# CompVis/ipoke

Measured on AMD Instinct MI355X. Metric: video-frames/sec (second-stage train step), higher is better.
Workload: dtype bf16; 1 GPU; plants_128 second_stage train, 16x3x128x128 clips, z=64, flow 2048 hidden (1.237 B params), per-GPU batch 20; global_batch=20, clip_frames=16, parallelism=dp1, weights=random init of the named architecture (no checkpoints offline)

## Files before the change

### include/ipoke_hip_dev.h

```cpp
#ifndef IPOKE_HIP_DEV_H
#define IPOKE_HIP_DEV_H

#include "ipoke_hip.h"

#ifdef __cplusplus
extern "C" {
#endif

int ipoke_conv_forward_repeat(const ipoke_conv_desc* d, int dtype, int n, void* stream);
int ipoke_set_dispatch_override(const char* name, int value);
enum { IPOKE_KERNEL_NONE = 0, IPOKE_KERNEL_IGEMM = 1, IPOKE_KERNEL_S8 = 2, IPOKE_KERNEL_HALO = 3, IPOKE_KERNEL_HALO16 = 4, IPOKE_KERNEL_C64 = 5, IPOKE_KERNEL_K8 = 6 };
int ipoke_last_conv_kernel(void);

int ipoke_spin_delay(int us, void* stream);

#define IPOKE_TAG_NT_SQUARE 1
#define IPOKE_TAG_TN_SQUARE 2
#define IPOKE_TAG_UNIT_FWD 3
#define IPOKE_TAG_UNIT_BWD 4
#define IPOKE_TAG_UNIT_INV 5
#define IPOKE_TAG_NN_SQUARE 6
#define IPOKE_TAG_CONV_BASE 16
#define IPOKE_TAG_WGRAD 32
int ipoke_timing_start(void);
int ipoke_timing_start_all(void);
int ipoke_timing_stop(const int* tags, int ntags, int* counts, double* mean_us);
int ipoke_timing_stop_ex(const int* tags, int ntags, int* counts, double* total_us, double* flops, double* bytes);

int ipoke_desc_sizes(int32_t* out, int n);

int ipoke_flow_test_inject_timeout(ipoke_flow* f, int which, void* stream);

int ipoke_gru_set_fused(int mode);

#ifdef __cplusplus
}
#endif
#endif
```

### ipoke_amd/_lib.py

```python
import ctypes
import os
from ctypes import CFUNCTYPE, POINTER, Structure, c_char_p, c_float, c_int, c_int32, c_int64, c_uint32, c_void_p

_HERE = os.path.dirname(os.path.abspath(__file__))
LIB_PATH = os.environ.get("IPOKE_LIB_PATH") or os.path.join(_HERE, "libipoke_hip.so")

F32, BF16 = 0, 1
ACT_NONE, ACT_ELU, ACT_RELU, ACT_LRELU02, ACT_TANH, ACT_SIGMOID = range(6)

DTYPES = {"f32": F32, "fp32": F32, "float32": F32, "bf16": BF16, "bfloat16": BF16}


class ConvDesc(Structure):
    _fields_ = [(n, c_int32) for n in ("NB", "Di", "Hi", "Wi", "Do", "Ho", "Wo", "kd", "kh", "kw", "sd", "sh", "sw",
                                       "pd", "ph", "pw", "transposed")] + [
        ("A", c_void_p), ("a_f32", c_int32),
        ("a_sn", c_int64), ("a_sd", c_int64), ("a_sh", c_int64), ("a_sw", c_int64), ("a_sc", c_int64),
        ("a_coff", c_int32), ("Kc_real", c_int32), ("Kc", c_int32),
        ("W", c_void_p), ("ldw", c_int32), ("Nout", c_int32),
        ("bias", c_void_p), ("act", c_int32), ("dact", c_void_p), ("ld_dact", c_int32), ("dact_act", c_int32),
        ("C", c_void_p), ("c_f32", c_int32), ("c_accumulate", c_int32), ("ldc", c_int64),
        ("c_coff", c_int32), ("c_cstride", c_int32), ("splitk", c_int32),
        ("c_scatter", c_int32), ("c_sn", c_int64), ("c_sh", c_int64), ("c_sw", c_int64), ("c_row0", c_int64),
        ("row_scale", c_void_p), ("rs_images", c_int32), ("rs_stride", c_int32), ("w_kmajor", c_int32), ("c_sd", c_int64),
# ... 148 lines not shown
    "ipoke_actnorm_logdet": (c_int, [_P, _P, c_int, c_int, _P, _P]),
    "ipoke_flow_nll": (c_int, [_P, _P, c_int, c_int, c_int, c_int, c_float, _P, _P, _P, _P]),
    "ipoke_adam_amsgrad_step": (c_int, [_P, _P, _P, _P, _P, c_int64, c_float, c_float, c_float, c_float, c_float, c_int,
                                        c_float, _P]),
    "ipoke_adam_amsgrad_step_grid": (c_int, [_P, _P, _P, _P, _P, c_int64, c_float, c_float, c_float, c_float, c_float, c_int,
                                             c_float, c_int, _P]),
    "ipoke_mcf_shadow_dims": (c_int, [c_int, c_int, c_int, POINTER(c_int32)]),
    "ipoke_mcf_fwd": (c_int, [POINTER(McfDesc), c_int, _P]),
    "ipoke_mcf_inv": (c_int, [POINTER(McfDesc), c_int, _P]),
    "ipoke_mcf_bwd": (c_int, [POINTER(McfDesc), c_int, _P]),
    "ipoke_macow_unit_supported": (c_int, [c_int, c_int, c_int]),
    "ipoke_macow_unit_xchg_bytes": (c_int64, [c_int, c_int]),
    "ipoke_macow_unit_fwd": (c_int, [POINTER(McfDesc), c_int, _P]),
    "ipoke_macow_unit_bwd": (c_int, [POINTER(McfDesc), c_int, _P]),
    "ipoke_macow_unit_inv": (c_int, [POINTER(McfDesc), c_int, _P]),
    "ipoke_relayout_job_size": (c_int, []),
    "ipoke_wn_job_size": (c_int, []),
    "ipoke_relayout_multi": (c_int, [_P, _P, _P, _P, c_int, c_int, _P, c_int, _P]),
    "ipoke_wn_scale_multi": (c_int, [_P, _P, _P, _P, c_int, c_int, _P]),
    "ipoke_wn_bwd_multi": (c_int, [_P, _P, _P, _P, c_int, c_int, _P]),
    "ipoke_groupnorm_workspace_floats": (c_int64, [c_int, c_int, c_int]),
    "ipoke_groupnorm": (c_int, [POINTER(NormDesc), c_int, _P]),
    "ipoke_add_act": (c_int, [_P, c_int, _P, c_int, _P, c_int, c_int64, c_int, c_int, c_int, _P]),
    "ipoke_gru_gates": (c_int, [_P, _P, c_int, _P, c_int, _P, c_int64, c_int, c_int, _P]),
    "ipoke_gru_update": (c_int, [_P, _P, _P, c_int, _P, c_int, c_int64, c_int, c_int, _P]),
    "ipoke_reparameterize": (c_int, [_P, c_int, _P, _P, _P, _P, c_int64, c_int, c_int, _P]),
    "ipoke_bilinear_cl": (c_int, [_P, _P, c_int, c_int, c_int, c_int, c_int, c_int, _P]),
    "ipoke_cl_to_nchw": (c_int, [_P, c_int, _P, c_int, c_int, c_int, c_int, _P]),
    "ipoke_nchw_to_cl": (c_int, [_P, _P, c_int, c_int, c_int, c_int, c_int, _P]),
    "ipoke_image_metrics_workspace_bytes": (c_int64, [c_int64, c_int, c_int]),
    "ipoke_psnr_ssim": (c_int, [_P, _P, c_int64, c_int, c_int, _P, _P, _P]),
    "ipoke_clip_to_cl4": (c_int, [_P, c_int64, c_int64, c_int64, c_int64, c_int64, c_int, c_int, c_int, c_int, c_int, c_int, _P, c_int, _P]),
    "ipoke_groupnorm_stats": (c_int, [_P, c_int, c_int, c_int, c_int, c_int, c_float, _P, c_int, _P]),
    "ipoke_groupnorm_stats_offset": (c_int64, [c_int, c_int, c_int]),
    "ipoke_groupnorm_bwd_workspace_floats": (c_int64, [c_int, c_int, c_int, c_int]),
    "ipoke_groupnorm_bwd": (c_int, [POINTER(NormBwdDesc), c_int, _P]),
    "ipoke_groupnorm_bwd_rs_workspace_floats": (c_int64, [c_int, c_int, c_int]),
    "ipoke_act_bwd": (c_int, [_P, c_int, _P, c_int, _P, c_int, c_int64, c_int, c_int, c_int, c_int, _P]),
    "ipoke_colsum_workspace_floats": (c_int64, [c_int64, c_int]),
    "ipoke_colsum": (c_int, [_P, c_int, c_int64, c_int, c_int, _P, c_int, _P, c_int, _P]),
    "ipoke_gru_update_bwd": (c_int, [_P, _P, _P, c_int, _P, c_int, _P, _P, _P, c_int, c_int64, c_int, c_int, _P]),
    "ipoke_gru_gates_bwd": (c_int, [_P, _P, c_int, _P, c_int, _P, _P, _P, c_int, c_int64, c_int, c_int, _P]),
    "ipoke_conv_weight_operand": (c_int, [_P, c_int, c_int, c_int, c_int, _P, _P, c_int, c_int, _P]),
    "ipoke_conv_weight_operand_multi": (c_int, [POINTER(c_void_p), POINTER(c_void_p), POINTER(c_int32), c_int, c_int, _P]),
    "ipoke_spectral_workspace_floats": (ctypes.c_long, [c_int, c_int, c_int]),
    "ipoke_spectral_sigma": (c_int, [_P, c_int, c_int, c_int, c_int, _P, _P, c_int, ctypes.c_float, _P, _P, _P, _P]),
    "ipoke_spectral_bwd": (c_int, [_P, c_int, c_int, c_int, c_int, _P, _P, _P, _P, _P]),
    "ipoke_spectral_bwd_workspace_floats": (ctypes.c_long, []),
    "ipoke_sn_job_size": (c_int, []),
    "ipoke_sn_jobs_upload": (c_int, [_P, c_int, _P, _P]),
    "ipoke_spectral_sigma_multi": (c_int, [_P, c_int, c_int, c_int, c_int, c_float, _P]),
    "ipoke_adam_multi": (c_int, [_P, _P, _P, _P, _P, c_int, ctypes.c_float, ctypes.c_float, ctypes.c_float, ctypes.c_float,
                                 ctypes.c_float, c_int, ctypes.c_float, _P]),
    "ipoke_maxpool3d_fwd": (c_int, [_P, _P, c_int, _P, c_int, _P, c_int, _P]),
    "ipoke_maxpool3d_bwd": (c_int, [_P, _P, c_int, _P, _P, c_int, c_int, _P]),
    "ipoke_avgpool_rows": (c_int, [_P, c_int, _P, c_int, c_int64, c_int, c_int, c_int, _P]),
    "ipoke_avgpool_rows_bwd": (c_int, [_P, c_int, _P, c_int, c_int64, c_int, c_int, c_int, _P]),
    "ipoke_groupnorm_jvp": (c_int, [_P, c_int, _P, c_int, _P, c_int, _P, c_int, _P, c_int, _P, c_int, c_int, c_int, c_int, c_int, c_float,
                                    _P, c_int, _P]),
    "ipoke_groupnorm_jvp_bwd": (c_int, [_P, c_int, _P, c_int, _P, c_int, _P, c_int, _P, c_int, _P, c_int, _P, c_int, _P, _P,
                                        c_int, c_int, c_int, c_int, c_int, c_float, _P, c_int, _P]),
    "ipoke_groupnorm_jvp_workspace_floats": (ctypes.c_long, [c_int, c_int]),
    "ipoke_gather_rows": (c_int, [_P, c_int, _P, _P, c_int, c_int64, c_int, c_int, _P]),
    "ipoke_l1_pair": (c_int, [_P, c_int, _P, c_int, c_int64, c_int, c_float, _P, _P, c_int, c_int, _P]),
    "ipoke_kl_loss": (c_int, [_P, _P, c_int64, c_int, _P, _P, _P, _P]),
    "ipoke_reparam_bwd": (c_int, [_P, c_int, _P, _P, _P, _P, _P, c_int, c_int64, c_int, c_int, _P]),
    "ipoke_l1_loss": (c_int, [_P, c_int, _P, c_int, c_int, c_int, c_int64, c_float, _P, _P, c_int, _P, _P]),
    "ipoke_l1_loss_partials": (ctypes.c_long, []),
    "ipoke_relayout_multi_range": (c_int, [_P, _P, _P, _P, c_int, c_int, c_int, _P, c_int, _P]),
    "ipoke_wn_scale_multi_range": (c_int, [_P, _P, _P, _P, c_int, c_int, c_int, c_int, _P]),
    "ipoke_flow_prepare_weights_range": (c_int, [_P, _P, _P, c_int64, c_int64, _P]),
    "ipoke_flow_set_native_adam": (c_int, [_P, _P, _P, _P, c_float, c_float, c_float, c_float, c_float, c_int, c_float, c_int]),
    "ipoke_flow_adam_range": (c_int, [_P, _P, _P, _P, _P, _P, _P, c_int64, c_int64, c_float, c_float, c_float, c_float, c_float, c_int,
                                      c_float, c_int, _P]),
    "ipoke_adam_tile_job_size": (c_int, []),
    "ipoke_adam_seg_size": (c_int, []),
    "ipoke_adam_amsgrad_shadow_tiles": (c_int, [_P, _P, _P, _P, _P, _P, _P, c_int, c_int, c_int, c_float, c_float, c_float, c_float, c_float,
                                                c_int, c_float, c_int, c_int, _P]),
    "ipoke_adam_amsgrad_cast_tiles": (c_int, [_P, _P, _P, _P, _P, _P, _P, c_int, c_int, c_int, c_float, c_float, c_float, c_float, c_float,
                                              c_int, c_float, c_int, c_int, _P]),
    "ipoke_adam_amsgrad_segments": (c_int, [_P, _P, _P, _P, _P, _P, c_int, c_int, c_int64, c_int64, c_float, c_float, c_float, c_float,
                                            c_float, c_int, c_float, c_int, _P]),
    "ipoke_wn_bwd_multi_range": (c_int, [_P, _P, _P, _P, c_int, c_int, c_int, c_int, _P]),
    "ipoke_flow_backward_pieces": (c_int, [_P, _P, _P, _P, _P, _P, c_int, _P, _P, _P, c_int, _P, GRAD_READY_FN, _P, _P]),
    "ipoke_video_to_cl": (c_int, [_P, c_int64, c_int64, c_int64, c_int64, c_int64, c_int, c_int, c_int, c_int, c_int, _P, c_int, c_int, c_int,
                                  c_int, _P, _P]),
    "ipoke_min_reset": (c_int, [_P, _P]),
    "ipoke_denorm_if_negative": (c_int, [_P, c_int64, c_int, c_int, c_int, c_int, _P, _P]),
    "ipoke_pool3d_same": (c_int, [_P, _P, c_int, _P, c_int, c_int, _P]),
    "ipoke_pool_rows_weighted": (c_int, [_P, c_int, _P, c_int, c_int64, c_int, c_int, _P, c_int, _P]),
    "ipoke_activation_moments": (c_int, [_P, c_int, c_int, _P, _P, _P, _P]),
    "ipoke_flow_resize": (c_int, [_P, _P, c_int, c_int, c_int, c_int, c_int, c_int, c_float, _P]),
    "ipoke_poke_workspace_bytes": (c_int64, [c_int, c_int, c_int, c_int, c_int]),
    "ipoke_poke_simulate": (c_int, [_P, c_int, c_int, c_int, c_int, c_int, c_int, c_int, _P, _P, _P, _P, _P, _P, _P, _P]),
    "ipoke_timing_start": (c_int, []),
    "ipoke_timing_start_all": (c_int, []),
    "ipoke_timing_stop": (c_int, [POINTER(c_int), c_int, POINTER(c_int), POINTER(ctypes.c_double)]),
    "ipoke_timing_stop_ex": (c_int, [POINTER(c_int), c_int, POINTER(c_int), POINTER(ctypes.c_double), POINTER(ctypes.c_double),
                                     POINTER(ctypes.c_double)]),
    "ipoke_flow_create": (c_int, [POINTER(FlowConfig), POINTER(c_void_p)]),
    "ipoke_flow_destroy": (None, [_P]),
    "ipoke_flow_piece_ranges": (c_int, [_P, c_int, POINTER(c_int64), c_int]),
    "ipoke_flow_handoff_timeouts": (c_int, [_P, POINTER(c_uint32)]),
    "ipoke_flow_side_stream": (c_void_p, [_P]),
    "ipoke_flow_test_inject_timeout": (c_int, [_P, c_int, _P]),
    "ipoke_conv_wgrad_splitm": (c_int, [_P, c_int, c_int]),
    "ipoke_conv_acc_scratch_bytes": (c_int64, [c_int, c_int, c_int]),
    "ipoke_conv_acc_scratch_init": (c_int, [_P, _P]),
    "ipoke_flow_param_count": (c_int64, [_P]),
    "ipoke_flow_index_count": (c_int64, [_P]),
    "ipoke_flow_tensor_count": (c_int32, [_P]),
    "ipoke_flow_op_count": (c_int32, [_P]),
    "ipoke_flow_tensor_info": (c_int, [_P, c_int, c_char_p, c_int, POINTER(c_int64), POINTER(c_int32), POINTER(c_int64),
                                       POINTER(c_int32)]),
    "ipoke_flow_shadow_bytes": (c_int64, [_P]),
    "ipoke_flow_set_graph": (c_int, [_P, c_int]),
    "ipoke_flow_float_buffer_count": (c_int64, [_P]),
    "ipoke_flow_set_float_buffers": (c_int, [_P, _P]),
    "ipoke_lu_job_size": (c_int, []),
    "ipoke_lu_prepare": (c_int, [_P, _P, _P, _P, c_int, _P]),
    "ipoke_lu_apply": (c_int, [_P, _P, c_int64, c_int, c_int, _P, c_int, _P]),
    "ipoke_lu_wgrad": (c_int, [_P, _P, c_int, c_int, c_int, _P, _P, _P, _P, _P, _P, _P]),
    "ipoke_flow_op_info": (c_int, [_P, c_int, POINTER(c_int64)]),
    "ipoke_flow_shadow_base": (c_int64, [_P]),
    "ipoke_flow_workspace_bytes": (c_int64, [_P, c_int, c_int]),
    "ipoke_flow_prepare_weights": (c_int, [_P, _P, _P, _P]),
    "ipoke_flow_forward": (c_int, [_P, _P, _P, _P, _P, _P, c_int, _P, _P, _P, c_int, _P]),
    "ipoke_flow_init_forward": (c_int, [_P, _P, _P, _P, c_int, _P, _P, _P, _P]),
    "ipoke_flow_reverse": (c_int, [_P, _P, _P, _P, _P, _P, c_int, _P, _P, _P]),
    "ipoke_flow_backward": (c_int, [_P, _P, _P, _P, _P, _P, c_int, _P, _P, _P, _P]),
}

_lib = None


def lib():
    global _lib
    if _lib is None:
        if not os.path.exists(LIB_PATH):
            raise RuntimeError(
                f"{LIB_PATH} not found: the HIP extension is not built. ipoke_amd has no CPU fallback; "
                "run `make -C ipoke_amd/csrc` (or __graft_entry__.build()) first.")
        import torch
        handle = ctypes.CDLL(LIB_PATH)
        for name, (res, args) in SIGNATURES.items():
            fn = getattr(handle, name)
            fn.restype = res
            fn.argtypes = args
        _lib = handle
    return _lib


def check(rc):
    if rc != 0:
        msg = lib().ipoke_last_error()
        raise RuntimeError(f"libipoke_hip call failed ({rc}): {msg.decode() if msg else '?'}")


def ptr(t):
    if t is None:
        return None
    return c_void_p(t.data_ptr())


def current_stream():
    import torch
# ... 23 lines not shown
```

### ipoke_amd/csrc/flow_engine.hip

```cpp
#include <functional>
#include <memory>
#include <vector>
#include <string>
#include <cstring>

#include "common.h"

namespace ipoke {

enum OpType { OP_ACTNORM = 0, OP_MCF = 1, OP_NICE = 2, OP_LU = 3 };
enum TensorKind { TK_PARAM = 0, TK_IDX_FWD = 1, TK_IDX_BWD = 2, TK_FLAG = 3, TK_FBUF = 4 };

struct TensorInfo {
  std::string name;
  int64_t offset;
  std::vector<int64_t> shape;
  int kind;
};

struct Op {
  int type = 0;
  int C = 0;
  int c0 = 0, Cn = 0;
  int64_t p_ls = -1, p_bias = -1, idx_fwd = -1, idx_bwd = -1;
  int order = 0;
  int64_t p_w1 = -1, p_b = -1, p_g = -1, p_v = -1;
  int Cp = 0, K1p = 0, K2p = 0, K3p = 0, Hq = 0, H = 0;
  int64_t sh_w1 = -1, sh_w1t = -1, sh_w2 = -1, sh_w2t = -1;
  int64_t wn_off = -1;
  int cin = 0, cout = 0, z_off = 0, z_stride = 1, t_off = 0, t_stride = 1;
  int64_t p_c1 = -1, p_c2 = -1;
  int Kc1 = 0, Kc3 = 0;
  int64_t sh_c1 = -1, sh_c1t = -1, sh_c2 = -1, sh_c2t = -1, sh_c3 = -1, sh_c3t = -1;
  int64_t ws_a = -1, ws_b = -1, ws_c = -1, ws_d = -1, ws_e = -1, ws_f = -1, ws_g = -1;
  int slot = -1;
  int mcf_idx = -1;
  int nice_idx = -1;
  int hidK = 0;
  int level = 0;
  int fuse_act = -1;
  bool fused = false;
  bool unit_head = false;
  int unit_of = -1;
  int lu_idx = -1;
  int an_next = -1;
  int an_prev = -1;
  int pair_unit = -1;
};

struct RelayoutJobH {
  long src_off, s_n, s_k, dstA, dstB, scale_off;
  int taps, n_real, k_real, A_rows_pad, A_inner_pad, B_rows_pad, B_inner_pad, B_rows_real, tile, tiles_k, block_start, frag_tiled;
};
struct WnJobH { long v_off, g_off, out_off; int rows, K, row_start; };
struct AdamTileJobH { long src_off, dstA, dstB; int N, K, tile_start, pad; };
struct AdamSegH { long off, len; };
struct LsRefH { long off; int C; };
struct LuJobH { long p_l, p_u, p_logs, b_perm, b_sign, b_lmask, b_umask, b_eye, w_off; int C, pad; };

}

using namespace ipoke;

struct ipoke_flow {
  ipoke_flow_config cfg;
  int esz = 2, e16 = 8, ks = 32;
  std::vector<TensorInfo> tensors;
  std::vector<Op> ops;
  int64_t n_params = 0, n_perm = 0, n_fbuf = 0;
  std::vector<LuJobH> lujobs; void* d_lujobs = nullptr; const float* fbuf = nullptr;
  int64_t shadow_elems = 0;
  int64_t wn_rows = 0;
  int nslots = 0;
  int n_mcf = 0;
  int tab_B = 0; void* d_w1tab = nullptr; void* d_w2tab = nullptr; void* d_redtab = nullptr; int n_red = 0;
  void* d_ntab[3] = {nullptr, nullptr, nullptr};
  int n_nice = 0;
  std::vector<RelayoutJobH> rjobs; int rblocks = 0;
  std::vector<AdamTileJobH> ajobs; int atiles = 0;
  std::vector<RelayoutJobH> rjobs2; int rblocks2 = 0;
  std::vector<AdamSegH> asegs;
  void* d_ajobs = nullptr; void* d_rjobs2 = nullptr; void* d_rblockjob2 = nullptr; void* d_asegs = nullptr;
  std::vector<WnJobH> wjobs;
  std::vector<LsRefH> lsrefs;
  void* d_rjobs = nullptr; void* d_wjobs = nullptr; void* d_lsrefs = nullptr; void* d_rblockjob = nullptr;
  hipStream_t side = nullptr;
  std::vector<hipStream_t> lanes;
  int n_lanes = 1;
  std::vector<hipEvent_t> events; size_t ev_next = 0;
  bool use_side = true;
  struct GraphEntry { std::vector<uintptr_t> key; hipGraph_t graph = nullptr; hipGraphExec_t exec = nullptr; int state = 0; uint64_t used = 0; };
  std::vector<GraphEntry> graphs; hipStream_t cap = nullptr; bool use_graph = false; uint64_t tick = 0;
  struct Unit { int64_t p_lo, p_hi; int wj_lo, wj_hi, row_lo, row_hi; int kind; int op_lo, op_hi; int64_t p2_lo = -1, p2_hi = -1; };
  std::vector<Unit> units;
  std::vector<int> red_first;
  int last_fwd_B = 0; bool have_saved = false;
  int P = 64;
  int unit_split = 1; void* d_xchg = nullptr;
  bool coupling_fuse = false; void* d_cxchg = nullptr;
  void* d_acc = nullptr; int64_t acc_bytes = 0;
  unsigned* h_tmo = nullptr; hipEvent_t pass_ev = nullptr; hipStream_t pass_stream = nullptr; bool pass_recorded = false, pass_unchecked = false;
  int64_t xchg_bytes = 0;
  bool mcf_xop = false;
  bool c2_straight = false;
  struct NativeAdam { bool on = false; float* m = nullptr; float* v = nullptr; float* vmax = nullptr; float lr = 0, beta1 = 0, beta2 = 0, eps = 0, wd = 0,
                      grad_scale = 1; int step = 0, max_blocks = 0; } nadam;
};

namespace {

int64_t align_up(int64_t v, int64_t a) { return (v + a - 1) / a * a; }

struct Builder {
  ipoke_flow& f;
  explicit Builder(ipoke_flow& fl) : f(fl) {}
  int64_t add_param(const std::string& name, std::vector<int64_t> shape) {
    int64_t n = 1; for (auto s : shape) n *= s;
    const int64_t off = f.n_params;
    f.tensors.push_back({name, off, shape, TK_PARAM});
    f.n_params = align_up(off + n, 4);
    return off;
  }
  int64_t add_idx(const std::string& name, int C, int kind) {
    const int64_t off = f.n_perm;
    f.tensors.push_back({name, off, {C}, kind});
    f.n_perm += C;
    return off;
  }
  void add_flag(const std::string& name) { f.tensors.push_back({name, -1, {}, TK_FLAG}); }
  int64_t add_fbuf(const std::string& name, std::vector<int64_t> shape) {
    int64_t n = 1; for (auto s : shape) n *= s;
    const int64_t off = f.n_fbuf;
    f.tensors.push_back({name, off, shape, TK_FBUF});
    f.n_fbuf = align_up(off + n, 4);
    return off;
  }
  void lu(const std::string& pfx, int C) {
    Op op; op.type = OP_LU; op.C = C; op.lu_idx = (int)f.lujobs.size();
    LuJobH j{};
    j.C = C;
    j.p_l = add_param(pfx + ".l", {C, C}); j.p_u = add_param(pfx + ".u", {C, C}); j.p_logs = add_param(pfx + ".log_s", {C});
    j.b_perm = add_fbuf(pfx + ".permutated", {C, C}); j.b_sign = add_fbuf(pfx + ".sign_s", {C});
    j.b_lmask = add_fbuf(pfx + ".lmask", {C, C}); j.b_umask = add_fbuf(pfx + ".umask", {C, C}); j.b_eye = add_fbuf(pfx + ".eye", {C, C});
    j.w_off = (long)op.lu_idx * 4 * 64 * 64;
    f.lujobs.push_back(j);
    f.lsrefs.push_back({j.p_logs, C});
    f.ops.push_back(op);
  }
  int64_t add_shadow(int64_t elems) {
    const int64_t off = f.shadow_elems;
    f.shadow_elems = align_up(off + elems, 64);
    return off;
  }
  void relayout_pair(long src, long s_n, long s_k, int taps, int n_real, int k_real, long scale, long dstA, int A_rows_pad,
                     int A_inner_pad, long dstB, int B_rows_pad, int B_inner_pad, int B_rows_real, int frag_tiled = 0) {
    const int tile = taps == 1 ? 64 : 32;
    const int n_ext = std::max(A_rows_pad, B_inner_pad), k_ext = std::max(A_inner_pad, B_rows_pad);
    const int tiles_n = (n_ext + tile - 1) / tile, tiles_k = (k_ext + tile - 1) / tile;
    RelayoutJobH j{src, s_n, s_k, dstA, dstB, scale, taps, n_real, k_real, A_rows_pad, A_inner_pad, B_rows_pad, B_inner_pad,
                   B_rows_real, tile, tiles_k, f.rblocks, frag_tiled};
    f.rjobs.push_back(j);
    f.rblocks += tiles_n * tiles_k;
    const bool fusable = taps == 1 && scale < 0 && !frag_tiled && s_k == 1 && s_n == k_real && n_real % 64 == 0 && k_real % 64 == 0 &&
                         A_rows_pad == n_real && A_inner_pad == k_real && B_rows_pad == k_real && B_inner_pad == n_real &&
                         B_rows_real == k_real;
    if (fusable) {
      f.ajobs.push_back({src, dstA, dstB, n_real, k_real, f.atiles, 0});
      f.atiles += (n_real / 64) * (k_real / 64);
    } else {
      j.block_start = f.rblocks2;
      f.rjobs2.push_back(j);
      f.rblocks2 += tiles_n * tiles_k;
    }
  }

  void actnorm(const std::string& pfx, int C_active, int c0, int Cn, const std::string* shuffle_pfx) {
    Op op; op.type = OP_ACTNORM; op.C = C_active; op.c0 = c0; op.Cn = Cn;
    if (!pfx.empty()) {
      op.p_ls = add_param(pfx + ".log_scale", {Cn, 1, 1});
      op.p_bias = add_param(pfx + ".bias", {Cn, 1, 1});
      add_flag(pfx + ".initialized");
      f.lsrefs.push_back({(long)op.p_ls, Cn});
    }
    if (shuffle_pfx) {
      op.idx_fwd = add_idx(*shuffle_pfx + ".forward_shuffle_idx", Cn, TK_IDX_FWD);
      op.idx_bwd = add_idx(*shuffle_pfx + ".backward_shuffle_idx", Cn, TK_IDX_BWD);
    }
    f.ops.push_back(op);
  }

  void mcf(const std::string& pfx, int C, int order) {
    const int Cc = f.cfg.cond_channels;
    Op op; op.type = OP_MCF; op.C = C; op.order = order;
    const int kh = order < 2 ? f.cfg.kernel_h : f.cfg.kernel_w, kw = order < 2 ? f.cfg.kernel_w : f.cfg.kernel_h;
    op.H = 4 * C;
    op.Cp = round_up(C, f.ks);
    op.K1p = 6 * op.Cp;
    op.K2p = round_up(op.H + Cc, f.ks);
    op.K3p = round_up(2 * C, f.ks);
    op.Hq = round_up(op.H, f.ks);
    const int K2 = op.H + Cc;
    op.p_w1 = add_param(pfx + ".net.shift_conv.weight", {op.H, C, kh, kw});
    add_flag(pfx + ".net.conv1x1.initialized");
    op.p_b = add_param(pfx + ".net.conv1x1.conv.bias", {2 * C});
    op.p_g = add_param(pfx + ".net.conv1x1.conv.weight_g", {2 * C, 1, 1, 1});
    op.p_v = add_param(pfx + ".net.conv1x1.conv.weight_v", {2 * C, K2, 1, 1});
    op.wn_off = f.wn_rows;
    f.wjobs.push_back({(long)op.p_v, (long)op.p_g, (long)op.wn_off, 2 * C, K2, (int)f.wn_rows});
    f.wn_rows += 2 * C;
    const int Hr = round_up(op.H, 16), N2r = round_up(2 * C, 16), Cr = round_up(C, 16);
    op.sh_w1 = add_shadow((int64_t)Hr * op.K1p);
    op.sh_w1t = add_shadow((int64_t)Cr * 6 * op.Hq);
    op.sh_w2 = add_shadow((int64_t)N2r * op.K2p);
    op.sh_w2t = add_shadow((int64_t)Hr * op.K3p);
    relayout_pair(op.p_w1, (long)C * 6, 6, 6, op.H, C, -1, op.sh_w1, Hr, op.Cp, op.sh_w1t, Cr, op.Hq, C, 1);
    relayout_pair(op.p_v, K2, 1, 1, 2 * C, K2, op.wn_off, op.sh_w2, N2r, op.K2p, op.sh_w2t, Hr, op.K3p, op.H, 1);
    op.slot = f.nslots++;
    op.mcf_idx = f.n_mcf++;
    f.ops.push_back(op);
  }

  void nice(const std::string& pfx, int C, bool skip, bool up, int factor) {
    const int hid = f.cfg.hidden;
    Op op; op.type = OP_NICE; op.C = C;
    op.cout = C / factor; op.cin = C - op.cout;
    if (skip && (C % 2 == 1)) skip = false;
    if (!skip) {
      const int z1 = up ? op.cin : op.cout;
      if (up) { op.z_off = 0; op.t_off = z1; } else { op.z_off = z1; op.t_off = 0; }
      op.z_stride = op.t_stride = 1;
    } else {
      op.z_stride = op.t_stride = 2;
      if (up) { op.z_off = 0; op.t_off = 1; } else { op.z_off = 1; op.t_off = 0; }
    }
    op.Kc1 = round_up(op.cin, f.e16);
    op.Kc3 = round_up(2 * op.cout, f.e16);
    const int hidK = hid + (f.cfg.condition_nice ? f.cfg.cond_channels : 0);
    op.hidK = hidK;
    op.p_c1 = add_param(pfx + ".net.conv1.weight", {hid, op.cin, 3, 3});
    op.p_c2 = add_param(pfx + ".net.conv2.weight", {hid, hid, 1, 1});
    add_flag(pfx + ".net.conv3.initialized");
    op.p_b = add_param(pfx + ".net.conv3.conv.bias", {2 * op.cout});
    op.p_g = add_param(pfx + ".net.conv3.conv.weight_g", {2 * op.cout, 1, 1, 1});
    op.p_v = add_param(pfx + ".net.conv3.conv.weight_v", {2 * op.cout, hidK, 3, 3});
    op.wn_off = f.wn_rows;
    f.wjobs.push_back({(long)op.p_v, (long)op.p_g, (long)op.wn_off, 2 * op.cout, hidK * 9, (int)f.wn_rows});
    f.wn_rows += 2 * op.cout;
    const int N3 = 2 * op.cout;
    op.sh_c1 = add_shadow((int64_t)hid * 9 * op.Kc1);
    op.sh_c1t = add_shadow((int64_t)op.cin * 9 * hid);
    op.sh_c2 = add_shadow((int64_t)hid * hid);
    op.sh_c2t = f.c2_straight ? -1 : add_shadow((int64_t)hid * hid);
    op.sh_c3 = add_shadow((int64_t)N3 * 9 * hidK);
// ... 331 lines not shown
    const int rmul = op.unit_of >= 0 || op.pair_unit >= 0 ? f->unit_split : 1;
    if (op.type == OP_MCF) {
      const McfGeom g = mcf_geom(op.order);
      w1[op.mcf_idx] = {f->mcf_xop ? (long)op.ws_e : (long)(plan.state0 + (int64_t)i * plan.state_stride), (long)op.ws_d, (long)op.p_w1, g.kh,
                        g.kw, -g.oy, -g.ox};
      w2[op.mcf_idx] = {(long)op.ws_a, (long)op.ws_c, (long)op.p_v, 1, 1, 0, 0};
      red.push_back({dbp, (long)op.p_b, 2 * op.C, 2 * op.C, rmul, 0});
    } else if (op.type == OP_NICE) {
      nt[0][op.nice_idx] = {(long)op.ws_g, (long)op.ws_f, (long)op.p_c1, 3, 3, 1, 1};
      nt[1][op.nice_idx] = {(long)op.ws_a, (long)op.ws_e, (long)op.p_c2, 1, 1, 0, 0, (long)op.sh_c2};
      nt[2][op.nice_idx] = {(long)op.ws_b, (long)op.ws_d, (long)op.p_v, 3, 3, 1, 1};
      red.push_back({dbp, (long)op.p_b, 2 * op.cout, 2 * op.cout, rmul, 0});
    } else if (op.p_ls >= 0) {
      red.push_back({dbp, (long)op.p_ls, 2 * op.Cn, op.Cn, rmul, 0});
      red.push_back({dbp + op.Cn, (long)op.p_bias, 2 * op.Cn, op.Cn, rmul, 0});
    }
  }
  drop_graphs(f);
  f->red_first[f->ops.size()] = (int)red.size();
  if (f->d_w1tab) { (void)hipFree(f->d_w1tab); (void)hipFree(f->d_w2tab); (void)hipFree(f->d_redtab); }
  for (int k = 0; k < 3; ++k) {
    if (f->d_ntab[k]) (void)hipFree(f->d_ntab[k]);
    IPK_HIP(hipMalloc(&f->d_ntab[k], nt[k].size() * sizeof(WgEntryH)));
    IPK_HIP(hipMemcpy(f->d_ntab[k], nt[k].data(), nt[k].size() * sizeof(WgEntryH), hipMemcpyHostToDevice));
  }
  IPK_HIP(hipMalloc(&f->d_w1tab, w1.size() * sizeof(WgEntryH)));
  IPK_HIP(hipMalloc(&f->d_w2tab, w2.size() * sizeof(WgEntryH)));
  IPK_HIP(hipMalloc(&f->d_redtab, red.size() * sizeof(RedEntryH)));
  IPK_HIP(hipMemcpy(f->d_w1tab, w1.data(), w1.size() * sizeof(WgEntryH), hipMemcpyHostToDevice));
  IPK_HIP(hipMemcpy(f->d_w2tab, w2.data(), w2.size() * sizeof(WgEntryH), hipMemcpyHostToDevice));
  IPK_HIP(hipMemcpy(f->d_redtab, red.data(), red.size() * sizeof(RedEntryH), hipMemcpyHostToDevice));
  f->n_red = (int)red.size();
  f->tab_B = B;
  return IPOKE_OK;
}

std::vector<std::pair<int, int>> backward_pieces(const ipoke_flow* f, int npieces) {
  std::vector<std::pair<int, int>> pieces;
  const int U = (int)f->units.size();
  int64_t total = 0;
  for (const auto& u : f->units) total += u.p_hi - u.p_lo;
  const int np = npieces < 1 ? 1 : (npieces > U ? U : npieces);
  static double ta = -1, tb = -1;
  if (ta < 0) {
    ta = 0.5; tb = 0.25;
    if (const char* e = getenv("IPOKE_PIECE_TAPER")) { double a = 0, b = 0; if (sscanf(e, "%lf,%lf", &a, &b) == 2 && a > 0 && b > 0) { ta = a; tb = b; } }
  }
  std::vector<double> w((size_t)np, 1.0);
  if (np >= 4) { w[(size_t)np - 2] = ta; w[(size_t)np - 1] = tb; }
  double wsum = 0; for (double x : w) wsum += x;
  int hi = U - 1;
  int64_t acc = 0; double target_acc = 0;
  int64_t done = 0;
  for (int u = U - 1; u >= 0; --u) {
    acc += f->units[u].p_hi - f->units[u].p_lo;
    const int idx = (int)pieces.size();
    const int left = np - idx;
    const double want = (double)total * (target_acc + w[(size_t)(idx < np ? idx : np - 1)]) / wsum;
    if (u == 0 || (left > 1 && ((double)(done + acc) >= want || u == left - 1))) {
      pieces.push_back({u, hi}); hi = u - 1; done += acc; acc = 0; target_acc += w[(size_t)(idx < np ? idx : np - 1)];
    }
  }
  return pieces;
}
void piece_param_ranges(const ipoke_flow* f, int lvl_lo, int lvl_hi, int64_t p0[3], int64_t p1[3]) {
  for (int k = 0; k < 3; ++k) { p0[k] = -1; p1[k] = -1; }
  for (int u = lvl_lo; u <= lvl_hi; ++u) {
    const auto& un = f->units[u];
    const int k = un.kind;
    if (p0[k] < 0) p0[k] = un.p_lo;
    p1[k] = un.p_hi;
    if (un.p2_lo >= 0) { if (p0[2] < 0) p0[2] = un.p2_lo; p1[2] = un.p2_hi; }
  }
}

hipEvent_t next_event(ipoke_flow* f) {
  hipEvent_t e = f->events[f->ev_next];
  f->ev_next = (f->ev_next + 1) % f->events.size();
  return e;
}

}

extern "C" int ipoke_flow_create(const ipoke_flow_config* cfg, ipoke_flow** out) {
  IPK_REQUIRE(cfg && out, "null argument");
  IPK_REQUIRE(cfg->dtype == IPOKE_F32 || cfg->dtype == IPOKE_BF16, "bad dtype");
  IPK_REQUIRE(cfg->n_levels >= 1 && cfg->n_levels <= 32 && cfg->n_levels < cfg->factor, "num_steps must be shorter than factor");
  IPK_REQUIRE(cfg->z_channels % cfg->factor == 0 && cfg->z_channels <= 64, "flow_in_channels must be a multiple of factor, <= 64");
  IPK_REQUIRE((cfg->z_channels / cfg->factor) % 2 == 0, "channel step must be even (skip split)");
  IPK_REQUIRE(cfg->kernel_h == 2 && cfg->kernel_w == 3, "kernel_size must be [2,3] (shipped configs)");
  IPK_REQUIRE(cfg->hidden % 32 == 0 && cfg->cond_channels % 32 == 0, "hidden / cond widths must be multiples of 32");
  std::unique_ptr<ipoke_flow> f(new ipoke_flow());
  f->cfg = *cfg;
  f->esz = cfg->dtype == IPOKE_BF16 ? 2 : 4; f->e16 = 16 / f->esz; f->ks = 64 / f->esz;
  {
    const char* cs = getenv("IPOKE_C2_STRAIGHT");
    f->c2_straight = cfg->dtype == IPOKE_BF16 && cfg->hidden % 64 == 0 && !(cs && cs[0] == '0');
  }
  int rc = build(*f); if (rc) return rc;
  {
    int64_t pos = 0;
    for (size_t k = 0; k < f->ajobs.size(); ++k) {
      IPK_REQUIRE(f->ajobs[k].src_off >= pos, "fused tensors must be in parameter order");
      if (f->ajobs[k].src_off > pos) f->asegs.push_back({(long)pos, (long)(f->ajobs[k].src_off - pos)});
      pos = f->ajobs[k].src_off + (int64_t)f->ajobs[k].N * f->ajobs[k].K;
    }
    if (pos < f->n_params) f->asegs.push_back({(long)pos, (long)(f->n_params - pos)});
    for (size_t k = 1; k < f->rjobs.size(); ++k) IPK_REQUIRE(f->rjobs[k].src_off > f->rjobs[k - 1].src_off, "relayout jobs must be in parameter order");
  }
  const char* env = getenv("IPOKE_NO_SIDE_STREAM");
  f->use_side = !(env && env[0] == '1');
  const char* gr = getenv("IPOKE_GRAPH");
  f->use_graph = gr && gr[0] == '1';
  const char* ln = getenv("IPOKE_LANES");
  f->n_lanes = ln ? atoi(ln) : 1;
  if (f->n_lanes < 1) f->n_lanes = 1;
  if (f->n_lanes > kMaxLanes) f->n_lanes = kMaxLanes;
  {
    const char* us = getenv("IPOKE_UNIT_SPLIT");
    f->unit_split = us ? atoi(us) : kDefaultUnitSplit;
    if (f->unit_split != 2 && f->unit_split != 4) f->unit_split = 1;
    if (f->n_lanes > 1 || cfg->dtype != IPOKE_BF16) f->unit_split = 1;
  }
  f->coupling_fuse = f->n_lanes == 1 && cfg->dtype == IPOKE_BF16 && ipoke_conv3x3_coupling_splitk(64, cfg->hidden, cfg->dtype) > 0;
  {
    const char* up = getenv("IPOKE_UNIT_PAIR");
    const bool on = f->unit_split > 1 && f->n_lanes == 1 && (up ? atoi(up) != 0 : true);
    for (size_t h = 2; on && h < f->ops.size(); ++h) {
      const Op& u = f->ops[h]; Op& an = f->ops[h - 1]; Op& cp = f->ops[h - 2];
      if (u.unit_head && an.type == OP_ACTNORM && an.an_prev == (int)h - 2 && cp.type == OP_NICE && an.c0 == 0 && an.Cn == u.C &&
          cp.cout <= 32 && cp.t_off + (cp.cout - 1) * cp.t_stride < u.C) {
        an.pair_unit = (int)h; cp.pair_unit = (int)h;
      }
    }
  }
  *out = f.release();
  return IPOKE_OK;
}

static int ensure_device(ipoke_flow* f) {
  if (f->d_rjobs) return IPOKE_OK;
  if (f->unit_split > 1 && !f->d_xchg) {
    const int64_t nb = ipoke_macow_unit_xchg_bytes(f->cfg.max_batch, f->unit_split);
    IPK_HIP(hipMalloc(&f->d_xchg, nb));
    IPK_HIP(hipMemset(f->d_xchg, 0, nb));
    f->xchg_bytes = nb;
  }
  if (!f->d_acc) {
    static const bool atomics = getenv("IPOKE_DGRAD_ATOMICS") != nullptr;
    if (!atomics) {
      f->acc_bytes = ipoke_conv_acc_scratch_bytes(f->cfg.max_batch * f->P, 64, 32);
      IPK_HIP(hipMalloc(&f->d_acc, (size_t)f->acc_bytes));
      int rc = ipoke_conv_acc_scratch_init(f->d_acc, nullptr); if (rc) return rc;
      IPK_HIP(hipDeviceSynchronize());
    }
  }
  if (!f->h_tmo) {
    IPK_HIP(hipHostMalloc(reinterpret_cast<void**>(&f->h_tmo), 64, hipHostMallocMapped));
    std::memset(f->h_tmo, 0, 64);
    IPK_HIP(hipEventCreateWithFlags(&f->pass_ev, hipEventDisableTiming));
  }
  if (f->coupling_fuse && !f->d_cxchg) {
    IPK_HIP(hipMalloc(&f->d_cxchg, (size_t)ipoke_conv3x3_coupling_xchg_bytes()));
    int rc = ipoke_conv3x3_coupling_xchg_init(f->d_cxchg, nullptr); if (rc) return rc;
    IPK_HIP(hipDeviceSynchronize());
  }
  IPK_REQUIRE((int)sizeof(RelayoutJobH) == ipoke_relayout_job_size() && (int)sizeof(WnJobH) == ipoke_wn_job_size(),
              "job table layout mismatch");
  IPK_HIP(hipMalloc(&f->d_rjobs, f->rjobs.size() * sizeof(RelayoutJobH)));
  IPK_HIP(hipMemcpy(f->d_rjobs, f->rjobs.data(), f->rjobs.size() * sizeof(RelayoutJobH), hipMemcpyHostToDevice));
  {
    std::vector<int32_t> bj((size_t)f->rblocks);
    for (size_t k = 0; k < f->rjobs.size(); ++k) {
      const int b0 = f->rjobs[k].block_start, b1 = k + 1 < f->rjobs.size() ? f->rjobs[k + 1].block_start : f->rblocks;
      for (int b = b0; b < b1; ++b) bj[b] = (int32_t)k;
    }
    IPK_HIP(hipMalloc(&f->d_rblockjob, bj.size() * sizeof(int32_t)));
    IPK_HIP(hipMemcpy(f->d_rblockjob, bj.data(), bj.size() * sizeof(int32_t), hipMemcpyHostToDevice));
  }
  IPK_REQUIRE((int)sizeof(AdamTileJobH) == ipoke_adam_tile_job_size() && (int)sizeof(AdamSegH) == ipoke_adam_seg_size(), "Adam table layout mismatch");
  if (!f->ajobs.empty()) {
    IPK_HIP(hipMalloc(&f->d_ajobs, f->ajobs.size() * sizeof(AdamTileJobH)));
    IPK_HIP(hipMemcpy(f->d_ajobs, f->ajobs.data(), f->ajobs.size() * sizeof(AdamTileJobH), hipMemcpyHostToDevice));
  }
  if (!f->asegs.empty()) {
    IPK_HIP(hipMalloc(&f->d_asegs, f->asegs.size() * sizeof(AdamSegH)));
    IPK_HIP(hipMemcpy(f->d_asegs, f->asegs.data(), f->asegs.size() * sizeof(AdamSegH), hipMemcpyHostToDevice));
  }
  if (!f->rjobs2.empty()) {
    IPK_HIP(hipMalloc(&f->d_rjobs2, f->rjobs2.size() * sizeof(RelayoutJobH)));
    IPK_HIP(hipMemcpy(f->d_rjobs2, f->rjobs2.data(), f->rjobs2.size() * sizeof(RelayoutJobH), hipMemcpyHostToDevice));
    std::vector<int32_t> bj((size_t)f->rblocks2);
    for (size_t k = 0; k < f->rjobs2.size(); ++k) {
      const int b0 = f->rjobs2[k].block_start, b1 = k + 1 < f->rjobs2.size() ? f->rjobs2[k + 1].block_start : f->rblocks2;
      for (int b = b0; b < b1; ++b) bj[b] = (int32_t)k;
    }
    IPK_HIP(hipMalloc(&f->d_rblockjob2, bj.size() * sizeof(int32_t)));
    IPK_HIP(hipMemcpy(f->d_rblockjob2, bj.data(), bj.size() * sizeof(int32_t), hipMemcpyHostToDevice));
  }
  IPK_HIP(hipMalloc(&f->d_wjobs, f->wjobs.size() * sizeof(WnJobH)));
  IPK_HIP(hipMemcpy(f->d_wjobs, f->wjobs.data(), f->wjobs.size() * sizeof(WnJobH), hipMemcpyHostToDevice));
  if (!f->lujobs.empty()) {
    IPK_REQUIRE((int)sizeof(LuJobH) == ipoke_lu_job_size(), "LU job table layout mismatch");
    IPK_HIP(hipMalloc(&f->d_lujobs, f->lujobs.size() * sizeof(LuJobH)));
    IPK_HIP(hipMemcpy(f->d_lujobs, f->lujobs.data(), f->lujobs.size() * sizeof(LuJobH), hipMemcpyHostToDevice));
  }
  IPK_HIP(hipMalloc(&f->d_lsrefs, f->lsrefs.size() * sizeof(LsRefH)));
  IPK_HIP(hipMemcpy(f->d_lsrefs, f->lsrefs.data(), f->lsrefs.size() * sizeof(LsRefH), hipMemcpyHostToDevice));
  {
    int least = 0, greatest = 0;
    IPK_HIP(hipDeviceGetStreamPriorityRange(&least, &greatest));
    static const bool flat = getenv("IPOKE_SIDE_FLAT_PRIORITY") != nullptr;
    IPK_HIP(hipStreamCreateWithPriority(&f->side, hipStreamNonBlocking, flat ? 0 : least));
  }
  IPK_HIP(hipStreamCreateWithFlags(&f->cap, hipStreamNonBlocking));
  f->lanes.resize(kMaxLanes - 1);
  for (auto& l : f->lanes) IPK_HIP(hipStreamCreateWithFlags(&l, hipStreamNonBlocking));
  f->events.resize(256);
  for (auto& e : f->events) IPK_HIP(hipEventCreateWithFlags(&e, hipEventDisableTiming));
  return IPOKE_OK;
}

extern "C" void ipoke_flow_destroy(ipoke_flow* f) {
  if (!f) return;
  if (f->d_rjobs) (void)hipFree(f->d_rjobs);
  if (f->d_wjobs) (void)hipFree(f->d_wjobs);
  if (f->d_lsrefs) (void)hipFree(f->d_lsrefs);
  if (f->d_lujobs) (void)hipFree(f->d_lujobs);
  if (f->d_rblockjob) (void)hipFree(f->d_rblockjob);
  if (f->d_ajobs) (void)hipFree(f->d_ajobs);
  if (f->d_asegs) (void)hipFree(f->d_asegs);
  if (f->d_rjobs2) (void)hipFree(f->d_rjobs2);
  if (f->d_rblockjob2) (void)hipFree(f->d_rblockjob2);
  if (f->d_w1tab) (void)hipFree(f->d_w1tab);
  for (int k = 0; k < 3; ++k) if (f->d_ntab[k]) (void)hipFree(f->d_ntab[k]);
  if (f->d_w2tab) (void)hipFree(f->d_w2tab);
  if (f->d_redtab) (void)hipFree(f->d_redtab);
  if (f->d_xchg) (void)hipFree(f->d_xchg);
  if (f->d_cxchg) (void)hipFree(f->d_cxchg);
  if (f->d_acc) (void)hipFree(f->d_acc);
  if (f->pass_ev) (void)hipEventDestroy(f->pass_ev);
  if (f->h_tmo) (void)hipHostFree(f->h_tmo);
  for (auto e : f->events) (void)hipEventDestroy(e);
  drop_graphs(f);
  if (f->side) (void)hipStreamDestroy(f->side);
  if (f->cap) (void)hipStreamDestroy(f->cap);
  for (auto l : f->lanes) if (l) (void)hipStreamDestroy(l);
  delete f;
}

extern "C" int ipoke_flow_piece_ranges(const ipoke_flow* f, int npieces, int64_t* ranges, int max_ranges) {
  IPK_REQUIRE(f != nullptr && (ranges != nullptr || max_ranges == 0), "bad arguments");
  const std::vector<std::pair<int, int>> pieces = backward_pieces(f, npieces);
  int n = 0;
  for (size_t i = 0; i < pieces.size(); ++i) {
    int64_t p0[3], p1[3];
    piece_param_ranges(f, pieces[i].first, pieces[i].second, p0, p1);
    for (int kind = 0; kind < 3; ++kind) {
      if (p0[kind] < 0 || p1[kind] <= p0[kind]) continue;
      if (n < max_ranges) { ranges[3 * n] = (int64_t)i; ranges[3 * n + 1] = p0[kind]; ranges[3 * n + 2] = p1[kind]; }
      ++n;
    }
  }
  return n;
}

extern "C" void* ipoke_flow_side_stream(ipoke_flow* f) {
  if (!f || ensure_device(f) != IPOKE_OK) return nullptr;
  return reinterpret_cast<void*>(f->side);
}
extern "C" int64_t ipoke_flow_param_count(const ipoke_flow* f) { return f ? f->n_params : -1; }
extern "C" int64_t ipoke_flow_index_count(const ipoke_flow* f) { return f ? f->n_perm : -1; }
extern "C" int ipoke_flow_set_graph(ipoke_flow* f, int enable) {
  IPK_REQUIRE(f != nullptr, "null flow handle");
  f->use_graph = enable != 0;
  return IPOKE_OK;
}
extern "C" int64_t ipoke_flow_float_buffer_count(const ipoke_flow* f) { return f ? f->n_fbuf : -1; }
extern "C" int ipoke_flow_set_float_buffers(ipoke_flow* f, const float* fbuf_dev) {
  IPK_REQUIRE(f != nullptr, "null flow handle");
  f->fbuf = fbuf_dev;
  return IPOKE_OK;
}
extern "C" int32_t ipoke_flow_tensor_count(const ipoke_flow* f) { return f ? (int32_t)f->tensors.size() : -1; }
extern "C" int32_t ipoke_flow_op_count(const ipoke_flow* f) { return f ? (int32_t)f->ops.size() : -1; }
extern "C" int ipoke_flow_tensor_info(const ipoke_flow* f, int i, char* name, int name_cap, int64_t* offset, int32_t* ndim,
                                      int64_t* shape4, int32_t* kind) {
  IPK_REQUIRE(f && i >= 0 && i < (int)f->tensors.size() && name && offset && ndim && shape4 && kind, "bad arguments");
  const TensorInfo& t = f->tensors[i];
  IPK_REQUIRE((int)t.name.size() + 1 <= name_cap, "name buffer too small");
  std::memcpy(name, t.name.c_str(), t.name.size() + 1);
  *offset = t.offset; *ndim = (int32_t)t.shape.size(); *kind = t.kind;
  for (int k = 0; k < 4; ++k) shape4[k] = k < (int)t.shape.size() ? t.shape[k] : 1;
  return IPOKE_OK;
}
extern "C" int ipoke_flow_op_info(const ipoke_flow* f, int i, int64_t* out32) {
  IPK_REQUIRE(f && out32 && i >= 0 && i < (int)f->ops.size(), "bad arguments");
  const Op& o = f->ops[i];
  const int64_t v[32] = {o.type, o.C, o.c0, o.Cn, o.p_ls, o.p_bias, o.idx_fwd, o.idx_bwd, o.order, o.p_w1, o.p_b, o.p_g, o.p_v,
                         o.sh_w1, o.sh_w1t, o.sh_w2, o.sh_w2t, o.wn_off, o.cin, o.cout, o.z_off, o.z_stride, o.t_off, o.t_stride,
                         o.p_c1, o.p_c2, o.sh_c1, o.sh_c1t, o.sh_c2, o.sh_c2t, o.sh_c3, o.sh_c3t};
  for (int k = 0; k < 32; ++k) out32[k] = v[k];
  return IPOKE_OK;
}
extern "C" int64_t ipoke_flow_shadow_base(const ipoke_flow* f) { return f ? 2 * align_up(f->wn_rows, 64) * 4 : -1; }

extern "C" int64_t ipoke_flow_shadow_bytes(const ipoke_flow* f) {
  if (!f) return -1;
  return 2 * align_up(f->wn_rows, 64) * 4 + f->shadow_elems * f->esz;
}
extern "C" int64_t ipoke_flow_workspace_bytes(ipoke_flow* f, int B, int training) {
  if (!f || B < 1) return -1;
  return make_plan(*f, B, training ? 1 : 0).bytes;
}
// ... 21 lines not shown
    const int row0 = f->wjobs[w0].row_start;
    const int row1 = w1 < (int)f->wjobs.size() ? f->wjobs[w1].row_start : (int)f->wn_rows;
    int rc = ipoke_wn_scale_multi_range(params, wn_scale, wn_inv, f->d_wjobs, w0, w1 - w0, row0, row1 - row0, stream);
    if (rc) return rc;
  }
  const std::vector<RelayoutJobH>& jobs = skip_fused ? f->rjobs2 : f->rjobs;
  const int nblocks = skip_fused ? f->rblocks2 : f->rblocks;
  int j0 = 0, j1 = 0;
  while (j0 < (int)jobs.size() && jobs[j0].src_off < begin) ++j0;
  j1 = j0;
  while (j1 < (int)jobs.size() && jobs[j1].src_off < end) ++j1;
  if (j1 > j0) {
    const int b0 = jobs[j0].block_start;
    const int b1 = j1 < (int)jobs.size() ? jobs[j1].block_start : nblocks;
    void* sh = reinterpret_cast<unsigned char*>(shadow) + 2 * align_up(f->wn_rows, 64) * 4;
    return ipoke_relayout_multi_range(params, sh, wn_scale, skip_fused ? f->d_rjobs2 : f->d_rjobs, (int)jobs.size(), b0, b1 - b0,
                                      reinterpret_cast<const int32_t*>(skip_fused ? f->d_rblockjob2 : f->d_rblockjob), f->cfg.dtype, stream);
  }
  return IPOKE_OK;
}

extern "C" int ipoke_flow_set_native_adam(ipoke_flow* f, float* m, float* v, float* vmax, float lr, float beta1, float beta2, float eps,
                                          float weight_decay, int step, float grad_scale, int max_blocks) {
  IPK_REQUIRE(f != nullptr, "null flow handle");
  ipoke_flow::NativeAdam& A = f->nadam;
  A.on = m != nullptr;
  if (!A.on) return IPOKE_OK;
  IPK_REQUIRE(v && vmax && step >= 1, "bad optimizer state");
  A.m = m; A.v = v; A.vmax = vmax; A.lr = lr; A.beta1 = beta1; A.beta2 = beta2; A.eps = eps; A.wd = weight_decay; A.step = step;
  A.grad_scale = grad_scale; A.max_blocks = max_blocks;
  return IPOKE_OK;
}

extern "C" int ipoke_flow_prepare_weights_range(ipoke_flow* f, const float* params, void* shadow, int64_t begin, int64_t end,
                                                void* stream) {
  IPK_REQUIRE(f && params && shadow && begin >= 0 && end >= begin, "bad arguments");
  { int rc0 = ensure_device(f); if (rc0) return rc0; }
  return prepare_range(f, params, shadow, begin, end, false, stream);
}

static int adam_range(ipoke_flow* f, float* params, const float* grads, float* m, float* v, float* vmax, void* shadow, int64_t begin, int64_t end,
                      float lr, float beta1, float beta2, float eps, float weight_decay, int step, float grad_scale, int max_blocks, void* stream,
                      bool skip_tiles = false);

extern "C" int ipoke_flow_adam_range(ipoke_flow* f, float* params, const float* grads, float* m, float* v, float* vmax, void* shadow,
                                     int64_t begin, int64_t end, float lr, float beta1, float beta2, float eps, float weight_decay,
                                     int step, float grad_scale, int max_blocks, void* stream) {
  IPK_REQUIRE(f && params && grads && m && v && vmax && shadow && begin >= 0 && end >= begin && end <= f->n_params, "bad arguments");
  { int rc0 = ensure_device(f); if (rc0) return rc0; }
  return adam_range(f, params, grads, m, v, vmax, shadow, begin, end, lr, beta1, beta2, eps, weight_decay, step, grad_scale, max_blocks, stream);
}

static int adam_range(ipoke_flow* f, float* params, const float* grads, float* m, float* v, float* vmax, void* shadow, int64_t begin, int64_t end,
                      float lr, float beta1, float beta2, float eps, float weight_decay, int step, float grad_scale, int max_blocks, void* stream,
                      bool skip_tiles) {
  if (end == begin) return IPOKE_OK;
  int a0 = 0, a1 = 0;
  while (a0 < (int)f->ajobs.size() && f->ajobs[a0].src_off < begin) ++a0;
  a1 = a0;
  while (a1 < (int)f->ajobs.size() && f->ajobs[a1].src_off < end) ++a1;
  if (a1 > a0 && !skip_tiles) {
    IPK_REQUIRE(f->ajobs[a1 - 1].src_off + (int64_t)f->ajobs[a1 - 1].N * f->ajobs[a1 - 1].K <= end, "range must cover whole tensors");
    const int t0 = f->ajobs[a0].tile_start, t1 = a1 < (int)f->ajobs.size() ? f->ajobs[a1].tile_start : f->atiles;
    void* sh = reinterpret_cast<unsigned char*>(shadow) + 2 * align_up(f->wn_rows, 64) * 4;
    int rc = f->c2_straight
        ? ipoke_adam_amsgrad_cast_tiles(params, grads, m, v, vmax, sh, f->d_ajobs, (int)f->ajobs.size(), t0, t1 - t0, lr, beta1, beta2,
                                        eps, weight_decay, step, grad_scale, max_blocks, f->cfg.dtype, stream)
        : ipoke_adam_amsgrad_shadow_tiles(params, grads, m, v, vmax, sh, f->d_ajobs, (int)f->ajobs.size(), t0, t1 - t0, lr, beta1, beta2,
                                          eps, weight_decay, step, grad_scale, max_blocks, f->cfg.dtype, stream);
    if (rc) return rc;
  }
  int s0 = 0, s1 = 0;
  while (s0 < (int)f->asegs.size() && f->asegs[s0].off + f->asegs[s0].len <= begin) ++s0;
  s1 = s0;
  while (s1 < (int)f->asegs.size() && f->asegs[s1].off < end) ++s1;
  if (s1 > s0) {
    int per = max_blocks > 0 ? max_blocks / (s1 - s0) : 16;
    if (per < 2) per = 2; if (per > 32) per = 32;
    int rc = ipoke_adam_amsgrad_segments(params, grads, m, v, vmax, f->d_asegs, s0, s1 - s0, begin, end, lr, beta1, beta2, eps, weight_decay,
                                         step, grad_scale, per, stream);
    if (rc) return rc;
  }
  return prepare_range(f, params, shadow, begin, end, true, stream);
}

static int make_lanes(const Ctx& full, int want, std::vector<Ctx>& lanes) {
  ipoke_flow* f = full.f;
  int n = want < 1 ? 1 : want;
  if (n > kMaxLanes) n = kMaxLanes;
  if (n > full.B) n = full.B;
  lanes.clear();
  int b0 = 0;
  for (int k = 0; k < n; ++k) {
    const int nb = (full.B - b0 + (n - k) - 1) / (n - k);
    Ctx c = full;
    c.b0 = b0; c.B = nb; c.M = (int64_t)nb * f->P; c.Bfull = full.B; c.lane = k;
    c.s = k == 0 ? full.s : f->lanes[k - 1];
    lanes.push_back(c);
    b0 += nb;
  }
  return IPOKE_OK;
}
static int fork_lanes(ipoke_flow* f, hipStream_t from, const std::vector<Ctx>& lanes) {
  if (lanes.size() < 2) return IPOKE_OK;
  hipEvent_t e = next_event(f);
  IPK_HIP(hipEventRecord(e, from));
  for (size_t k = 1; k < lanes.size(); ++k) IPK_HIP(hipStreamWaitEvent(lanes[k].s, e, 0));
  return IPOKE_OK;
}
static int join_lanes(ipoke_flow* f, const std::vector<Ctx>& lanes, hipStream_t to) {
  for (size_t k = 0; k < lanes.size(); ++k) {
    if (lanes[k].s == to) continue;
    hipEvent_t e = next_event(f);
    IPK_HIP(hipEventRecord(e, lanes[k].s));
    IPK_HIP(hipStreamWaitEvent(to, e, 0));
  }
  return IPOKE_OK;
}

template <typename Fn>
static int with_graph(ipoke_flow* f, std::vector<uintptr_t> key, hipStream_t caller, Fn enqueue) {
  if (!f->use_graph) return enqueue(caller);
  int rc0 = ensure_device(f); if (rc0) return rc0;
  ipoke_flow::GraphEntry* e = nullptr;
  for (auto& g : f->graphs) if (g.key == key) { e = &g; break; }
  if (!e) {
    if (f->graphs.size() >= 12) {
      size_t old = 0;
      for (size_t i = 1; i < f->graphs.size(); ++i) if (f->graphs[i].used < f->graphs[old].used) old = i;
      if (f->graphs[old].exec) (void)hipGraphExecDestroy(f->graphs[old].exec);
      if (f->graphs[old].graph) (void)hipGraphDestroy(f->graphs[old].graph);
      f->graphs.erase(f->graphs.begin() + old);
    }
    ipoke_flow::GraphEntry ne; ne.key = std::move(key); ne.used = ++f->tick;
    f->graphs.push_back(std::move(ne));
    return enqueue(caller);
  }
  e->used = ++f->tick;
  if (e->state < 0) return enqueue(caller);
  if (!e->exec) {
    const std::vector<uintptr_t> k = e->key;
    IPK_HIP(hipStreamBeginCapture(f->cap, hipStreamCaptureModeThreadLocal));
    const int rc = enqueue(f->cap);
    hipGraph_t g = nullptr;
    const hipError_t er = hipStreamEndCapture(f->cap, &g);
    e = nullptr;
    for (auto& ge : f->graphs) if (ge.key == k) { e = &ge; break; }
    if (rc != IPOKE_OK) { if (g) (void)hipGraphDestroy(g); if (e) e->state = -1; return rc; }
    if (er != hipSuccess || !g || !e) { (void)hipGetLastError(); if (g) (void)hipGraphDestroy(g); if (e) e->state = -1; return enqueue(caller); }
    hipGraphExec_t ex = nullptr;
    if (hipGraphInstantiate(&ex, g, nullptr, nullptr, 0) != hipSuccess) {
      (void)hipGetLastError(); (void)hipGraphDestroy(g); e->state = -1; return enqueue(caller);
    }
    e->graph = g; e->exec = ex; e->state = 1;
  }
  hipEvent_t a = next_event(f);
  IPK_HIP(hipEventRecord(a, caller)); IPK_HIP(hipStreamWaitEvent(f->cap, a, 0));
  IPK_HIP(hipGraphLaunch(e->exec, f->cap));
  hipEvent_t b = next_event(f);
  IPK_HIP(hipEventRecord(b, f->cap)); IPK_HIP(hipStreamWaitEvent(caller, b, 0));
  return IPOKE_OK;
}

__global__ void handoff_poll_kernel(const unsigned* unit_xchg, const unsigned* coupling_xchg, unsigned* host_words) {
  if (threadIdx.x == 0) {
    host_words[0] = unit_xchg ? unit_xchg[0] : 0u;
// ... 349 lines not shown
  auto wgrads_wait_lanes = [&]() -> int {
    int r0 = join_lanes(f, lanes, ws_stream); if (r0) return r0;
    if (side_delay > 0 && f->use_side) return ipoke_spin_delay(side_delay, wstream);
    return IPOKE_OK;
  };
  rc = ensure_tables(f, B, c.plan); if (rc) return rc;
  int pend_lo = -1, pend_hi = -1, pend_op = -1;
  auto flush_mcf = [&]() -> int {
    if (pend_lo < 0) return IPOKE_OK;
    const Op& op = f->ops[pend_op];
    const int nb = pend_hi - pend_lo + 1;
    int r = wgrads_wait_lanes(); if (r) return r;
    static const int mcf_cap = getenv("IPOKE_TN_MAX_WGS") ? atoi(getenv("IPOKE_TN_MAX_WGS")) : 0;
    ipoke_wgrad_desc w; std::memset(&w, 0, sizeof(w));
    w.NB = B; w.Di = 1; w.Hi = 8; w.Wi = 8; w.Do = 1; w.Ho = 8; w.Wo = 8; w.kd = w.kh = w.kw = 1; w.sd = w.sh = w.sw = 1;
    w.max_workgroups = f->use_side ? mcf_cap : 0;
    const int K2 = op.H + f->cfg.cond_channels;
    w.a_f32 = 0; w.a_sn = 64L * op.K2p; w.a_sh = 8L * op.K2p; w.a_sw = op.K2p; w.a_sc = 1; w.Kc_real = K2; w.Kc = op.K2p;
    w.ldy = op.K3p; w.Nout = 2 * op.C; w.w_sn = K2; w.w_sc = 1; w.w_st = 0;
    r = ipoke_conv_wgrad_batched(&w, reinterpret_cast<const unsigned char*>(f->d_w2tab) + (size_t)pend_lo * ipoke_wgrad_batch_entry_size(),
                                 nb, c.ws, c.ws, grads, c.dtype, wstream);
    if (r) return r;
    std::memset(&w, 0, sizeof(w));
    w.NB = B; w.Di = 1; w.Hi = 8; w.Wi = 8; w.Do = 1; w.Ho = 8; w.Wo = 8; w.kd = 1; w.kh = 2; w.kw = 3; w.sd = w.sh = w.sw = 1;
    w.max_workgroups = f->use_side ? mcf_cap : 0;
    if (f->mcf_xop) {
      w.a_f32 = 0; w.a_sn = 64L * op.Cp; w.a_sh = 8L * op.Cp; w.a_sw = op.Cp; w.a_sc = 1; w.Kc_real = op.Cp; w.Kc = op.Cp; w.Kc_store = op.C;
    } else {
      w.a_f32 = 1; w.a_sn = 64L * c.ld; w.a_sh = 8L * c.ld; w.a_sw = c.ld; w.a_sc = 1; w.Kc_real = op.C; w.Kc = op.Cp;
    }
    w.ldy = op.Hq; w.Nout = op.H; w.w_sn = (int64_t)op.C * 6; w.w_sc = 6; w.w_st = 1;
    r = ipoke_conv_wgrad_batched(&w, reinterpret_cast<const unsigned char*>(f->d_w1tab) + (size_t)pend_lo * ipoke_wgrad_batch_entry_size(),
                                 nb, c.ws, c.ws, grads, c.dtype, wstream);
    pend_lo = pend_hi = pend_op = -1;
    return r;
  };
  if (f->use_side) {
    hipEvent_t e = next_event(f);
    IPK_HIP(hipEventRecord(e, s)); IPK_HIP(hipStreamWaitEvent(f->side, e, 0));
  }
  hipStream_t rs = ready_stream ? ready_stream : s;
  const std::vector<std::pair<int, int>> pieces = backward_pieces(f, npieces);
  const int wgrad_adam_mode = getenv("IPOKE_WGRAD_ADAM") ? atoi(getenv("IPOKE_WGRAD_ADAM")) : 0;
  const bool wgrad_adam = wgrad_adam_mode != 0 && f->nadam.on && !getenv("IPOKE_PROBE_SKIP_ADAM") && f->c2_straight &&
                          c.dtype == IPOKE_BF16 && f->use_side && lanes.size() == 1 && hid % 128 == 0 && (int)f->ajobs.size() == f->n_nice && !f->cfg.condition_nice;
  std::function<int()> flush_nice_fn = []() { return (int)IPOKE_OK; };
  auto native_adam_range = [&](int64_t b0, int64_t b1, int max_blocks) -> int {
    const ipoke_flow::NativeAdam& A = f->nadam;
    float* pm = const_cast<float*>(params);
    void* rstream = reinterpret_cast<void*>(rs);
    if (f->c2_straight)
      return adam_range(f, pm, grads, A.m, A.v, A.vmax, const_cast<void*>(shadow), b0, b1, A.lr, A.beta1, A.beta2, A.eps, A.wd, A.step,
                        A.grad_scale, max_blocks, rstream, wgrad_adam);
    int r = ipoke_adam_amsgrad_step_grid(pm + b0, grads + b0, A.m + b0, A.v + b0, A.vmax + b0, b1 - b0, A.lr, A.beta1, A.beta2, A.eps, A.wd, A.step,
                                         A.grad_scale, max_blocks, rstream);
    if (r) return r;
    return prepare_range(f, params, const_cast<void*>(shadow), b0, b1, false, rstream);
  };
  auto finish_piece = [&](int lvl_lo, int lvl_hi, int piece) -> int {
    int r = flush_nice_fn(); if (r) return r;
    r = flush_mcf(); if (r) return r;
    r = join_lanes(f, lanes, rs); if (r) return r;
    if (f->use_side && f->side != rs) {
      hipEvent_t e = next_event(f);
      IPK_HIP(hipEventRecord(e, f->side)); IPK_HIP(hipStreamWaitEvent(rs, e, 0));
    }
    void* rstream = reinterpret_cast<void*>(rs);
    const int r0 = f->red_first[f->units[lvl_lo].op_lo], r1 = f->red_first[f->units[lvl_hi].op_hi];
    if (r1 > r0) {
      r = ipoke_reduce_rows_multi(reinterpret_cast<const float*>(c.ws), grads,
                                  reinterpret_cast<const unsigned char*>(f->d_redtab) + (size_t)r0 * ipoke_reduce_entry_size(), r1 - r0, B,
                                  rstream);
      if (r) return r;
    }
    int64_t p0[3] = {-1, -1, -1}, p1[3] = {-1, -1, -1};
    int wj0[3] = {0, 0, 0}, wj1[3] = {0, 0, 0}, rw0[3] = {0, 0, 0}, rw1[3] = {0, 0, 0};
    for (int u = lvl_lo; u <= lvl_hi; ++u) {
      const auto& un = f->units[u];
      const int k = un.kind;
      if (p0[k] < 0) { p0[k] = un.p_lo; wj0[k] = un.wj_lo; rw0[k] = un.row_lo; }
      p1[k] = un.p_hi; wj1[k] = un.wj_hi; rw1[k] = un.row_hi;
      if (un.p2_lo >= 0) { if (p0[2] < 0) p0[2] = un.p2_lo; p1[2] = un.p2_hi; }
    }
    for (int kind = 0; kind < 2; ++kind) {
      if (p0[kind] < 0) continue;
      r = ipoke_wn_bwd_multi_range(params, grads, c.wn_inv(), f->d_wjobs, wj0[kind], wj1[kind] - wj0[kind], rw0[kind],
                                   rw1[kind] - rw0[kind], rstream);
      if (r) return r;
    }
    static const bool probe_skip_adam = getenv("IPOKE_PROBE_SKIP_ADAM") != nullptr;
    if (f->nadam.on && !probe_skip_adam) {
      ipoke_flow::NativeAdam A = f->nadam;
      {
        static const int early = getenv("IPOKE_ADAM_EARLY_BLOCKS") ? atoi(getenv("IPOKE_ADAM_EARLY_BLOCKS")) : 0;
        static const int late = getenv("IPOKE_ADAM_LATE_PIECES") ? atoi(getenv("IPOKE_ADAM_LATE_PIECES")) : 3;
        if (early > 0 && piece < (int)pieces.size() - late) A.max_blocks = early;
      }
      for (int kind = 0; kind < 3; ++kind) {
        if (p0[kind] < 0 || p1[kind] <= p0[kind]) continue;
        r = native_adam_range(p0[kind], p1[kind], A.max_blocks); if (r) return r;
      }
    }
    if (ready)
      for (int kind = 0; kind < 3; ++kind)
        if (p0[kind] >= 0 && p1[kind] > p0[kind]) ready(user, piece, p0[kind], p1[kind]);
    return IPOKE_OK;
  };
  std::vector<int> pend_nice;
  auto flush_nice = [&]() -> int {
    if (pend_nice.empty()) return IPOKE_OK;
    int rc = wgrads_wait_lanes(); if (rc) return rc;
    static const int tn_cap = getenv("IPOKE_TN_MAX_WGS") ? atoi(getenv("IPOKE_TN_MAX_WGS")) : 0;
    size_t i0 = 0;
    while (i0 < pend_nice.size()) {
      const Op& op = f->ops[pend_nice[i0]];
      size_t i1 = i0 + 1;
      while (i1 < pend_nice.size()) {
        const Op& o2 = f->ops[pend_nice[i1]];
        if (o2.nice_idx != f->ops[pend_nice[i1 - 1]].nice_idx - 1 || o2.Kc1 != op.Kc1 || o2.cin != op.cin || o2.cout != op.cout ||
            o2.Kc3 != op.Kc3) break;
        ++i1;
      }
      const int nb = (int)(i1 - i0), lo = f->ops[pend_nice[i1 - 1]].nice_idx;
      ipoke_wgrad_desc w;
      auto base8 = [&](int k, int pad) {
        std::memset(&w, 0, sizeof(w));
        w.NB = B; w.Di = 1; w.Hi = 8; w.Wi = 8; w.Do = 1; w.Ho = 8; w.Wo = 8; w.kd = 1; w.kh = w.kw = k;
        w.sd = w.sh = w.sw = 1; w.ph = w.pw = pad;
        w.max_workgroups = f->use_side ? tn_cap : 0;
      };
      auto entries = [&](int k) {
        return reinterpret_cast<const unsigned char*>(f->d_ntab[k]) + (size_t)lo * ipoke_wgrad_batch_entry_size();
      };
      base8(3, 1);
      w.a_sn = 64L * op.hidK; w.a_sh = 8L * op.hidK; w.a_sw = op.hidK; w.a_sc = 1; w.Kc_real = op.hidK; w.Kc = op.hidK;
      w.ldy = op.Kc3; w.Nout = 2 * op.cout;
      w.w_sn = (int64_t)op.hidK * 9; w.w_sc = 9; w.w_st = 1;
      rc = ipoke_conv_wgrad_batched(&w, entries(2), nb, c.ws, c.ws, grads, c.dtype, wstream); if (rc) return rc;
      base8(1, 0);
      w.a_sn = 64L * hid; w.a_sh = 8L * hid; w.a_sw = hid; w.a_sc = 1; w.Kc_real = hid; w.Kc = hid;
      w.ldy = hid; w.Nout = hid;
      w.w_sn = hid; w.w_sc = 1; w.w_st = 0;
      ipoke_wgrad_adam wa;
      if (wgrad_adam) {
        const ipoke_flow::NativeAdam& A = f->nadam;
        wa.params = const_cast<float*>(params); wa.m = A.m; wa.v = A.v; wa.vmax = A.vmax;
        wa.operand = const_cast<unsigned char*>(c.shadow + c.shadow_base());
        wa.lr = A.lr; wa.beta1 = A.beta1; wa.beta2 = A.beta2; wa.eps = A.eps; wa.weight_decay = A.wd; wa.grad_scale = A.grad_scale; wa.step = A.step;
        wa.keep_grad = wgrad_adam_mode == 2;
        w.adam = &wa;
      }
      rc = ipoke_conv_wgrad_batched(&w, entries(1), nb, c.ws, c.ws, grads, c.dtype, wstream); if (rc) return rc;
      base8(3, 1);
      w.a_f32 = 0; w.a_sn = 64L * op.Kc1; w.a_sh = 8L * op.Kc1; w.a_sw = op.Kc1; w.a_sc = 1;
      w.Kc_real = op.Kc1; w.Kc = op.Kc1;
      w.ldy = hid; w.Nout = hid;
      w.w_sn = (int64_t)op.cin * 9; w.w_sc = 9; w.w_st = 1; w.Kc_store = op.cin;
      rc = ipoke_conv_wgrad_batched(&w, entries(0), nb, c.ws, c.ws, grads, c.dtype, wstream); if (rc) return rc;
      i0 = i1;
    }
    pend_nice.clear();
    return IPOKE_OK;
  };
  flush_nice_fn = flush_nice;
  static const int flush_min = getenv("IPOKE_NICE_FLUSH_MIN") ? atoi(getenv("IPOKE_NICE_FLUSH_MIN")) : 4;
  auto maybe_flush_nice = [&]() -> int { return (int)pend_nice.size() >= flush_min ? flush_nice() : (int)IPOKE_OK; };
  size_t pk = 0;
  int cur = 0;
  int pending_an = -1;
  const int64_t goff[2] = {c.plan.g0, c.plan.g1};
  for (int i = (int)f->ops.size() - 1; i >= 0; --i) {
    const Op& op = f->ops[i];
    if (op.unit_of >= 0 && i == op.unit_of + 5) {
      const int h = op.unit_of;
      rc = maybe_flush_nice(); if (rc) return rc;
      static const int lidx[4] = {0, 1, 3, 4};
      for (const Ctx& l : lanes) {
        ipoke_mcf_desc d4[4];
        for (int k = 0; k < 4; ++k) {
          const int j = h + lidx[k];
          const Op& mk = f->ops[j];
          mcf_desc(l, mk, d4[k]);
          d4[k].x = l.state(j);
// ... 164 lines not shown
```

### ipoke_amd/csrc/gemm.hip

```cpp
#include "common.h"
#include <atomic>
#include <cstring>
#include <mutex>
#include <type_traits>

namespace ipoke {

static constexpr int kPitch = 144;

struct GeomDev {
  int M;
  int lDo, lHo, lWo;
  int Do, Ho, Wo, pow2, S;
  int Di, Hi, Wi;
  int khw, kw, taps;
  int sd, sh, sw, pd, ph, pw;
  int lsd, lsh, lsw;
  int transposed;
};

struct NtParams {
  GeomDev g;
  const void* A; int a_f32; long a_sn, a_sd, a_sh, a_sw, a_sc; int a_coff, Kc_real, Kc;
  const void* W; int ldw; int Nout; int Ktot;
// ... 2214 lines not shown
    if (nfrag == 0) continue;
    const unsigned char* ab = abuf + buf * ABUF;
    for (int t = 0; t < ntaps; ++t) {
      const int ta = t / g.kw, tb = t - ta * g.kw;
      const int dy = g.transposed ? g.ph - ta : ta - g.ph, dx = g.transposed ? g.pw - tb : tb - g.pw;
      const int sr0 = (wm * 4 + 1 + dy) * HW + (lane & 15) + 1 + dx;
      const unsigned char* wb = wbuf + (t * nch + ch) * 64 * 128;
#pragma unroll
      for (int hs = 0; hs < 2; ++hs) {
        frag_t fa[MREP], fb[NREP];
#pragma unroll
        for (int i = 0; i < MREP; ++i) {
          const int sr = sr0 + i * HW;
          fa[i] = *reinterpret_cast<const frag_t*>(ab + sr * 128 + (((hs * 4 + qlo) ^ ((sr >> 1) & 7)) * 16));
        }
#pragma unroll
        for (int j = 0; j < NREP; ++j) fb[j] = *reinterpret_cast<const frag_t*>(wb + (b_rd[j] ^ (hs * 64)));
#if IPOKE_C64_ABL == 1
#pragma unroll
        for (int i = 0; i < MREP; ++i) asm volatile("" :: "v"(fa[i]), "v"(fb[0]), "v"(fb[1]));
#else
#pragma unroll
        for (int i = 0; i < MREP; ++i) {
          GEMM_MMA(fa[i], fb[0], acc[i][0]);
          if (nfrag > 1) GEMM_MMA(fa[i], fb[1], acc[i][1]);
        }
#endif
      }
    }
    if (ch + 1 < nch) continue;
#if IPOKE_C64_ABL == 2
    if (v >= 0) { asm volatile("" :: "v"(acc[0][0]), "v"(acc[1][0]), "v"(acc[2][0]), "v"(acc[3][0]), "v"(acc[0][1]), "v"(acc[1][1]), "v"(acc[2][1]), "v"(acc[3][1])); continue; }
#endif
    const int tile = v / nch;
    const int tx = tile % tiles_x, t2 = tile / tiles_x, ty = t2 % tiles_y, img = t2 / tiles_y;
    const int oy = ty * TH + wm * 4, ox = tx * TW + (lane & 15);
    const float img_scale = image_scale(p, img);
#pragma unroll
    for (int j = 0; j < NREP; ++j) {
      const int n = wn * 32 + j * 16 + qlo * 4;
      if (j >= nfrag || n >= p.n_pad) continue;
      const bool full = vec_ok && n + 3 < p.Nout;
      f32x4 b4 = f32x4{0.f, 0.f, 0.f, 0.f};
      if (p.bias) {
        if (full) b4 = *reinterpret_cast<const f32x4*>(p.bias + n);
        else for (int e = 0; e < 4; ++e) if (n + e < p.Nout) b4[e] = p.bias[n + e];
      }
#pragma unroll
      for (int i = 0; i < MREP; ++i) {
        const long m = p.c_scatter ? p.c_row0 + (long)img * p.c_sn + (long)(oy + i) * p.c_sh + (long)ox * p.c_sw
                                   : ((long)img * g.Ho + oy + i) * g.Wo + ox;
        f32x4 v4 = acc[i][j] * img_scale + b4;
        if (p.act != IPOKE_ACT_NONE) {
#pragma unroll
          for (int e = 0; e < 4; ++e) v4[e] = fast_act<T>(p.act, v4[e]);
        }
        if (!full) {
#pragma unroll
          for (int e = 0; e < 4; ++e) if (n + e >= p.Nout) v4[e] = 0.f;
        }
        if (p.c_f32) {
          float* Cp = reinterpret_cast<float*>(p.C) + m * p.ldc + p.c_coff;
          if (full && p.c_cstride == 1 && ((p.ldc | p.c_coff) & 3) == 0) *reinterpret_cast<f32x4*>(Cp + n) = v4;
          else for (int e = 0; e < 4; ++e) if (n + e < p.Nout) Cp[(long)(n + e) * p.c_cstride] = v4[e];
        } else {
          T* Cp = reinterpret_cast<T*>(p.C) + m * p.ldc + p.c_coff + n;
          if (n + 3 < p.n_pad && ((p.ldc | p.c_coff) & 3) == 0) {
            pack_t o;
#pragma unroll
            for (int e = 0; e < 4; ++e) o[e] = ET<T>::from_f32(v4[e]);
            *reinterpret_cast<pack_t*>(Cp) = o;
          } else {
            for (int e = 0; e < 4; ++e)
              if (n + e < p.n_pad) Cp[e] = ET<T>::from_f32(v4[e]);
          }
        }
      }
    }
  }
  wait_vmcnt<0>();
}

static std::atomic<int> g_c64_mode{-1}, g_halo16_mode{-1};
static int dispatch_mode(std::atomic<int>& slot, const char* env_name) {
  int m = slot.load(std::memory_order_relaxed);
  if (m < 0) {
    const char* e = getenv(env_name);
    m = e ? atoi(e) : 1;
    if (m < 0 || m > 2) m = 1;
    int expect = -1;
    if (!slot.compare_exchange_strong(expect, m)) m = expect;
  }
  return m;
}

static bool c64_applicable(const NtParams& p) {
  const int mode = dispatch_mode(g_c64_mode, "IPOKE_C64");
  const GeomDev& g = p.g;
  if (!mode) return false;
  const int kh = g.kw > 0 ? g.khw / g.kw : 0;
  const int lo_y = g.transposed ? g.ph - (kh - 1) : -g.ph, hi_y = g.transposed ? g.ph : kh - 1 - g.ph;
  const int lo_x = g.transposed ? g.pw - (g.kw - 1) : -g.pw, hi_x = g.transposed ? g.pw : g.kw - 1 - g.pw;
  const int nch = p.Kc / 64;
  const bool can = !p.a_f32 && !p.dact && g.taps == g.khw && kh >= 1 && g.khw == kh * g.kw && g.Di == 1 && g.Do == 1 && g.pd == 0 &&
                   g.Hi == g.Ho && g.Wi == g.Wo && g.Ho % 16 == 0 && g.Wo % 16 == 0 && g.sd == 1 && g.sh == 1 && g.sw == 1 &&
                   lo_y >= -1 && hi_y <= 1 && lo_x >= -1 && hi_x <= 1 && (!g.transposed || (kh == 3 && g.kw == 3)) &&
                   (p.Kc == 64 || p.Kc == 128) && p.Kc_real == p.Kc && g.khw * nch <= 9 && (g.khw > 1 || p.c_scatter) && p.Nout <= 64 && (p.a_coff & 7) == 0 &&
                   p.ldw >= p.Ktot && (p.ldw & 7) == 0 && p.splitk == 1 && !p.c_acc && ((p.a_sn | p.a_sh | p.a_sw) & 7) == 0 && p.n_pad <= 64 &&
                   (reinterpret_cast<uintptr_t>(p.W) & 15) == 0;
  if (!can || kLdsC64 > device_max_lds()) return false;
  return mode == 2 || g.M / 256 >= 512;
}
static int launch_conv3x3_c64(NtParams& p, hipStream_t s) {
  const size_t lds = kLdsC64;
  auto kern = conv3x3_c64_kernel;
  IPK_SET_LDS_ONCE(kern, lds);
  const int ntiles = p.g.M / 256;
  p.tiles_m = ntiles; p.tiles_n = 1; p.xa = p.xb = 0;
  hipLaunchKernelGGL(kern, dim3((unsigned)std::min(ntiles, 256)), dim3(512), lds, s, p);
  IPK_LAUNCH_CHECK();
  return IPOKE_OK;
}

static bool halo16_applicable(const NtParams& p) {
  const int mode = dispatch_mode(g_halo16_mode, "IPOKE_HALO16");
  const GeomDev& g = p.g;
  static const bool phase_on = !(getenv("IPOKE_HALO16_PHASE") && atoi(getenv("IPOKE_HALO16_PHASE")) == 0);
  const bool phase4 = phase_on && g.taps == 4 && g.khw == 4 && g.kw == 2 && g.ph == 0 && g.pw == 0 && !g.transposed && g.Di == 1 && g.Do == 1 && g.pd == 0 &&
                      g.sd == 1 && p.c_scatter && !p.dact;
  if (!mode || p.a_f32) return false;
  if (!phase4 && (p.c_scatter || !(g.taps == 9 || g.taps == 27) || g.khw != 9 || g.kw != 3)) return false;
  const bool flat = phase4 || (g.taps == 9 && g.Di == 1 && g.Do == 1 && g.pd == 0 && g.sd == 1);
  const bool deep = !phase4 && g.taps == 27 && g.pd == 1 && (p.a_sd & 7) == 0 && (g.sd == 1 ? g.Di == g.Do : (!g.transposed && g.sd == 2));
  if (!(flat || deep)) return false;
  const bool can = g.Hi == g.Ho && g.Wi == g.Wo && g.Ho % 16 == 0 && g.Wo % 16 == 0 && g.sh == 1 && g.sw == 1 && (phase4 || (g.ph == 1 && g.pw == 1)) &&
                   p.Kc % 64 == 0 && p.Kc_real == p.Kc && (p.a_coff & 7) == 0 && p.ldw >= p.Ktot && p.splitk == 1 && !p.c_acc &&
                   ((p.a_sn | p.a_sh | p.a_sw) & 7) == 0 &&
                   (long)(g.M / g.S) * p.a_sn + (long)g.Di * p.a_sd + (long)g.Hi * p.a_sh + p.Kc < (1L << 31) && (long)p.Nout * p.ldw < (1L << 31);
  if (!can || kLdsHalo16 > device_max_lds()) return false;
  if (mode == 2) return true;
  const long wgs = (long)(g.M / 256) * ceil_div(p.Nout, 128), rounds = (wgs + 255) / 256;
  const bool shallow = deep && g.Do <= 2 && g.Di <= 2 * g.sd;
  return (deep ? p.Kc >= 64 : p.Kc >= 128) && p.Nout >= 96 && wgs >= 256 && (wgs * 10 >= rounds * 256 * 8 || (shallow && wgs * 10 >= rounds * 256 * 6));
}
static int launch_conv3x3_halo16(NtParams& p, hipStream_t s) {
  const size_t lds = kLdsHalo16;
  auto kern = conv3x3_halo16_kernel;
  IPK_SET_LDS_ONCE(kern, lds);
  p.tiles_m = p.g.M / 256; p.tiles_n = ceil_div(p.Nout, 128); p.xa = p.xb = 0;
  dim3 grid((unsigned)p.tiles_m, (unsigned)p.tiles_n);
  hipLaunchKernelGGL(kern, grid, dim3(512), lds, s, p);
  IPK_LAUNCH_CHECK();
  return IPOKE_OK;
}

static bool halo_applicable(const NtParams& p) {
  static const int on = getenv("IPOKE_HALO") ? atoi(getenv("IPOKE_HALO")) : 1;
  const GeomDev& g = p.g;
  static const int on3 = getenv("IPOKE_HALO3D") ? atoi(getenv("IPOKE_HALO3D")) : 1;
  const bool flat = g.taps == 9 && g.Di == 1 && g.Do == 1 && g.pd == 0;
  const bool deep = on3 && g.taps == 27 && g.Di == g.Do && g.pd == 1 && (p.a_sd & 7) == 0;
  if (!(flat || deep) || p.c_scatter || kLdsHalo > device_max_lds()) return false;
  if (deep) {
    if (p.Kc > 64) return false;
    return on && !p.a_f32 && g.khw == 9 && g.kw == 3 && g.Hi == g.Ho && g.Wi == g.Wo && g.Ho % 8 == 0 && g.Wo % 16 == 0 &&
           g.sd == 1 && g.sh == 1 && g.sw == 1 && g.ph == 1 && g.pw == 1 && p.Kc % 64 == 0 && p.Kc_real == p.Kc && (p.a_coff & 7) == 0 &&
// ... 1342 lines not shown
  }
  if (p.splitm < 1) p.splitm = 1;
  if (p.splitm > nmb) p.splitm = nmb;
  p.mb_per_split = ceil_div(nmb, p.splitm);
  if constexpr (sizeof(T) == 2) {
    if (lat8_applicable(p, nbatch)) return launch_lat8(p, s, nbatch);
    if (nbatch == 1 && halo_wgrad_applicable(p)) return launch_halo_wgrad(p, s);
  }
  const size_t lds = 4 * 128 * kPitch + 256 * sizeof(int);
  static const int glds = getenv("IPOKE_TN_GLDS") ? atoi(getenv("IPOKE_TN_GLDS")) : 1;
  if (glds && sizeof(T) == 2 && !p.a_f32 && p.a_sc == 1 && (p.a_coff & 7) == 0 && (p.Kc & 7) == 0 &&
      (p.ldy & 7) == 0 && (p.y_coff & 7) == 0 && ((p.a_sn | p.a_sd | p.a_sh | p.a_sw) & 7) == 0 &&
      (p.batch ? ((reinterpret_cast<uintptr_t>(p.a_base) | reinterpret_cast<uintptr_t>(p.y_base)) & 15) == 0
               : ((reinterpret_cast<uintptr_t>(p.A) | reinterpret_cast<uintptr_t>(p.dY)) & 15) == 0)) {
    static const int nst = getenv("IPOKE_TN_STAGES") ? atoi(getenv("IPOKE_TN_STAGES")) : 2;
    const int NST = nst == 3 ? 3 : 2;
    static const int narrow_on = getenv("IPOKE_TN_NARROW") ? atoi(getenv("IPOKE_TN_NARROW")) : 1;
    const bool narrow = narrow_on && NST == 2 && p.batch != nullptr && p.Nout <= 64 && p.Ktot >= 512 && p.max_wgs <= 0;
    if (narrow) p.tiles_k = ceil_div(p.Ktot, 256);
    const int nst_n = narrow_on == 3 ? 3 : 2;
    const size_t lds2 = narrow ? (size_t)nst_n * 3 * 64 * 256 + 256 * sizeof(int) : (size_t)NST * 2 * 64 * 256 + 256 * sizeof(int);
    const bool adam = p.ad_p != nullptr;
    if (adam) IPK_REQUIRE(!narrow && p.batch && p.g.taps == 1 && p.w_sc == 1 && p.w_sn == p.Ktot && p.Nout % 128 == 0 && p.Ktot % 128 == 0 &&
                          p.splitm == 1 && !p.accumulate && p.Kc == p.Kc_real && (p.Kc_store == 0 || p.Kc_store == p.Kc) && (p.w_sn & 3) == 0,
                          "Adam in the weight-gradient epilogue: batched dense 1x1 problems in whole 128 x 128 tiles, one reduction split");
    auto kern = adam ? (NST == 2 ? igemm_tn_glds_kernel<2, 64, false, true> : igemm_tn_glds_kernel<3, 64, false, true>)
                : narrow ? (nst_n == 3 ? igemm_tn_glds_kernel<3, 64, true> : igemm_tn_glds_kernel<2, 64, true>)
                       : NST == 2 ? igemm_tn_glds_kernel<2, 64> : igemm_tn_glds_kernel<3, 64>;
    if (adam && NST == 2) { IPK_SET_LDS_ONCE(kern, lds2); } else if (adam) { IPK_SET_LDS_ONCE(kern, lds2); }
    else if (narrow && nst_n == 3) { IPK_SET_LDS_ONCE(kern, lds2); } else if (narrow) { IPK_SET_LDS_ONCE(kern, lds2); }
    else if (NST == 2) { IPK_SET_LDS_ONCE(kern, lds2); } else { IPK_SET_LDS_ONCE(kern, lds2); }
    const int ntiles = p.tiles_n * p.tiles_k;
    const int cap = p.max_wgs > 0 ? p.max_wgs : ntiles;
    p.xa = p.xb = 0;
    static const bool xcd_map = !(getenv("IPOKE_TN_XCD") && atoi(getenv("IPOKE_TN_XCD")) == 0);
    if (xcd_map && cap >= ntiles && ntiles % 8 == 0) {
      double best = -1;
      for (int xa = 1; xa <= 8; xa *= 2) {
        const int xb = 8 / xa;
        if (p.tiles_n % xa || p.tiles_k % xb) continue;
        const double cost = (double)p.tiles_n / xa + (double)p.tiles_k / xb;
        if (best < 0 || cost < best) { best = cost; p.xa = xa; p.xb = xb; }
      }
    }
    for (int t0 = 0; t0 < ntiles; t0 += cap) {
      p.tile0 = t0;
      const int nt = std::min(cap, ntiles - t0);
      const int zper = p.max_wgs > 0 ? std::max(1, p.max_wgs / std::max(1, nt * p.splitm)) : nbatch;
      for (int z0 = 0; z0 < nbatch; z0 += zper) {
        p.z0 = z0;
        dim3 grid2((unsigned)nt, (unsigned)p.splitm, (unsigned)std::min(zper, nbatch - z0));
        hipLaunchKernelGGL(kern, grid2, dim3(512), lds2, s, p);
        IPK_LAUNCH_CHECK();
      }
    }
    return IPOKE_OK;
  }
  IPK_REQUIRE(p.ad_p == nullptr, "Adam in the weight-gradient epilogue needs the LDS-DMA kernel (bf16, dense 16-byte aligned operands)");
  static const int nr = getenv("IPOKE_TN_NR") ? atoi(getenv("IPOKE_TN_NR")) : 2;
  dim3 grid((unsigned)(p.tiles_n * p.tiles_k), (unsigned)p.splitm, (unsigned)nbatch);
  if (nr == 2) {
    auto kern = igemm_tn_kernel<T, 2>;
    IPK_SET_LDS_ONCE(kern, lds);
    hipLaunchKernelGGL(kern, grid, dim3(256), lds, s, p);
  } else {
    auto kern = igemm_tn_kernel<T, 4>;
    IPK_SET_LDS_ONCE(kern, lds);
    hipLaunchKernelGGL(kern, grid, dim3(256), lds, s, p);
  }
  IPK_LAUNCH_CHECK();
  return IPOKE_OK;
}

}

using namespace ipoke;

#ifdef IPOKE_GEMM_STAMPS
extern "C" void ipoke_gemm_set_stamps(long long* base) { g_gemm_stamps = base; }
#endif

extern "C" int ipoke_set_dispatch_override(const char* name, int value) {
  IPK_REQUIRE(name != nullptr && value <= 2, "bad arguments");
  std::atomic<int>* slot = !strcmp(name, "c64") ? &g_c64_mode : (!strcmp(name, "halo16") ? &g_halo16_mode : nullptr);
  IPK_REQUIRE(slot != nullptr, "unknown dispatch switch (c64 | halo16)");
  slot->store(value < 0 ? -1 : value, std::memory_order_relaxed);
  return IPOKE_OK;
}

extern "C" int ipoke_last_conv_kernel(void) { return g_last_kernel; }

namespace ipoke {
static int conv_params(NtParams& p, const ipoke_conv_desc* d, int dtype) {
  IPK_REQUIRE(d != nullptr, "null descriptor");
  IPK_REQUIRE(dtype == IPOKE_F32 || dtype == IPOKE_BF16, "bad dtype");
  const int esz = dtype == IPOKE_BF16 ? 2 : 4, e16 = 16 / esz;
  int rc = make_geom(p.g, d->NB, d->Di, d->Hi, d->Wi, d->Do, d->Ho, d->Wo, d->kd, d->kh, d->kw, d->sd, d->sh, d->sw,
                     d->pd, d->ph, d->pw, d->transposed);
  if (rc) return rc;
  IPK_REQUIRE(d->A && d->W && d->C, "null tensor");
  IPK_REQUIRE(d->Kc % e16 == 0 && d->Kc >= d->Kc_real && d->Kc_real > 0, "Kc must be a padded multiple of 16 bytes");
  if (!d->a_f32) {
    IPK_REQUIRE(d->a_sc == 1, "dtype activations must be channels-last");
    IPK_REQUIRE(d->Kc_real % e16 == 0 && d->a_coff % e16 == 0, "dtype activations need 16-byte aligned channel runs");
    IPK_REQUIRE(d->a_sn % e16 == 0 && d->a_sd % e16 == 0 && d->a_sh % e16 == 0 && d->a_sw % e16 == 0,
                "dtype activations need 16-byte aligned rows");
    IPK_REQUIRE(((uintptr_t)d->A & 15) == 0, "A must be 16-byte aligned");
  }
  IPK_REQUIRE(d->ldw % e16 == 0 && ((uintptr_t)d->W & 15) == 0, "weights need 16-byte aligned rows");
  IPK_REQUIRE(d->w_kmajor ? d->ldw >= d->Nout : (d->ldw >= round_up(p.g.taps * d->Kc, e16) || d->ldw >= p.g.taps * d->Kc), "ldw too small");
  p.A = d->A; p.a_f32 = d->a_f32; p.a_sn = d->a_sn; p.a_sd = d->a_sd; p.a_sh = d->a_sh; p.a_sw = d->a_sw; p.a_sc = d->a_sc;
  p.a_coff = d->a_coff; p.Kc_real = d->Kc_real; p.Kc = d->Kc;
  p.W = d->W; p.ldw = d->ldw; p.Nout = d->Nout; p.Ktot = p.g.taps * d->Kc;
  p.bias = d->bias; p.act = d->act; p.dact = d->dact; p.ld_dact = d->ld_dact; p.dact_act = d->dact_act;
  p.C = d->C; p.c_f32 = d->c_f32; p.c_acc = d->c_accumulate; p.ldc = d->ldc; p.c_coff = d->c_coff;
  p.c_cstride = d->c_cstride <= 0 ? 1 : d->c_cstride;
  p.splitk = d->splitk < 1 ? 1 : d->splitk;
  p.c_scatter = d->c_scatter; p.c_sn = d->c_sn; p.c_sd = d->c_sd; p.c_sh = d->c_sh; p.c_sw = d->c_sw; p.c_row0 = d->c_row0;
  p.row_scale = d->row_scale; p.rs_images = d->rs_images; p.rs_stride = d->rs_stride < 1 ? 1 : d->rs_stride;
  if (d->row_scale) IPK_REQUIRE(p.splitk == 1 && !d->c_accumulate && d->rs_images >= 1, "row scale: plain stores, rs_images >= 1");
  if (d->c_scatter) IPK_REQUIRE(p.splitk == 1 && !d->dact && !d->c_accumulate && d->c_row0 >= 0 && (p.g.Do == 1 || d->c_sd > 0), "output scatter: plain stores; maps with depth need c_sd");
  p.n_pad = d->Nout;
  if (!d->c_f32 && p.splitk == 1) {
    const long lim = d->ldc - d->c_coff;
    p.n_pad = (int)(round_up(d->Nout, e16) < lim ? round_up(d->Nout, e16) : lim);
  }
  p.acc_cnt = nullptr; p.acc_part = nullptr; p.acc_part_bytes = 0;
  if (p.splitk > 1 && d->c_accumulate) {
    IPK_REQUIRE(d->c_f32 && !d->bias && d->act == IPOKE_ACT_NONE && !d->dact, "split-K accumulates raw fp32 sums only");
    if (d->acc_scratch) {
      IPK_REQUIRE(((uintptr_t)d->acc_scratch & 15) == 0 && d->acc_scratch_bytes > kAccCounterBytes && d->Nout <= 64,
                  "bad accumulation scratch (16-byte aligned, ipoke_conv_acc_scratch_bytes; Nout <= 64)");
      p.acc_cnt = reinterpret_cast<unsigned*>(d->acc_scratch);
      p.acc_part = reinterpret_cast<float*>(reinterpret_cast<unsigned char*>(d->acc_scratch) + kAccCounterBytes);
      p.acc_part_bytes = d->acc_scratch_bytes - kAccCounterBytes;
    }
  } else if (p.splitk > 1) {
    IPK_REQUIRE(d->ldc % 4 == 0 && d->ldc >= d->Nout, "split-K partials need ldc >= Nout, multiple of 4");
  } else if (!d->c_f32) {
    IPK_REQUIRE(p.c_cstride == 1 && !d->c_accumulate, "dtype outputs are dense, non-accumulating");
  }
  return IPOKE_OK;
}
}

extern "C" int ipoke_conv_forward(const ipoke_conv_desc* d, int dtype, void* stream) {
  NtParams p;
  int rc = conv_params(p, d, dtype); if (rc) return rc;
  const int esz = dtype == IPOKE_BF16 ? 2 : 4;
  hipStream_t s = reinterpret_cast<hipStream_t>(stream);
  {
    static const int prio = getenv("IPOKE_NT_PRIO") ? atoi(getenv("IPOKE_NT_PRIO")) : 2;
    p.prio = prio;
  }
#ifdef IPOKE_GEMM_STAMPS
  p.stamps = g_gemm_stamps;
  if (g_gemm_stamps) g_gemm_stamps += 4 * 4096;
#endif
  const bool square = p.g.taps == 1 && d->Nout == p.Ktot && d->Nout >= 1024 && p.splitk == 1;
  TimedScope ts(square ? (d->w_kmajor ? IPOKE_TAG_NN_SQUARE : IPOKE_TAG_NT_SQUARE) : IPOKE_TAG_CONV_BASE, s);
  p.w_kmajor = d->w_kmajor;
  static const bool clog = getenv("IPOKE_CONV_LOG") != nullptr;
  hipEvent_t le0 = nullptr, le1 = nullptr;
  if (clog) { IPK_HIP(hipEventCreate(&le0)); IPK_HIP(hipEventCreate(&le1)); IPK_HIP(hipEventRecord(le0, s)); }
  if (p.w_kmajor) {
    IPK_REQUIRE(dtype == IPOKE_BF16, "K-major weights: bf16 only (the f32 mode keeps its transposed shadows)");
    g_last_kernel = IPOKE_KERNEL_IGEMM;
    rc = dispatch_nn(p, s);
// ... 133 lines not shown
```

### ipoke_amd/csrc/prep.hip

```cpp
#include "common.h"

namespace ipoke {

struct RelayoutJob {
  long src_off;
  long s_n, s_k;
  long dstA, dstB;
  long scale_off;
  int taps, n_real, k_real;
  int A_rows_pad, A_inner_pad, B_rows_pad, B_inner_pad, B_rows_real;
  int tile, tiles_k;
  int block_start;
  int frag_tiled;
};

template <typename T>
__device__ __forceinline__ long tiled_offset(int row, int col, int ld) {
  constexpr int KS = 64 / (int)sizeof(T), E16 = 16 / (int)sizeof(T);
  const int rb = row >> 4, r = row & 15, ks = col / KS, cq = col - ks * KS;
  return ((long)rb * (ld / KS) + ks) * (16 * KS) + (cq / E16) * (16 * E16) + r * E16 + (cq % E16);
}

template <typename T> struct RPack4;
template <> struct RPack4<bf16_t> { typedef __attribute__((ext_vector_type(4))) __bf16 type; };
template <> struct RPack4<float> { typedef f32x4 type; };

template <typename T, int TAPS, int TE>
__device__ __forceinline__ void relayout_tile(const RelayoutJob& j, const float* __restrict__ params, T* __restrict__ shadow,
                                              const float* __restrict__ wn_scale, int n0, int k0, float* tile) {
  constexpr int TP = TE + 1;
  constexpr int total = TE * TE * TAPS;
  typedef typename RPack4<T>::type pack_t;
  const bool k_mid = j.s_k < j.s_n;
  if (TAPS == 1 && j.s_k == 1 && ((j.s_n | j.src_off) & 3) == 0) {
    for (int e = threadIdx.x; e < total / 4; e += 256) {
      const int kl = (e % (TE / 4)) * 4, nl = e / (TE / 4);
      const int n = n0 + nl, k = k0 + kl;
      f32x4 v = {0.f, 0.f, 0.f, 0.f};
      if (n < j.n_real && k < j.k_real) {
        if (k + 3 < j.k_real) {
          v = *reinterpret_cast<const f32x4*>(params + j.src_off + (long)n * j.s_n + k);
        } else {
          for (int q = 0; q < 4; ++q) if (k + q < j.k_real) v[q] = params[j.src_off + (long)n * j.s_n + k + q];
        }
        if (j.scale_off >= 0) { const float sc = wn_scale[j.scale_off + n]; v[0] *= sc; v[1] *= sc; v[2] *= sc; v[3] *= sc; }
      }
#pragma unroll
      for (int q = 0; q < 4; ++q) tile[nl * TP + kl + q] = v[q];
    }
  } else {
    for (int e = threadIdx.x; e < total; e += 256) {
      const int t = e % TAPS, rest = e / TAPS;
      const int m = rest % TE, sl = rest / TE;
      const int nl = k_mid ? sl : m, kl = k_mid ? m : sl;
      const int n = n0 + nl, k = k0 + kl;
      float v = 0.f;
      if (n < j.n_real && k < j.k_real) {
        v = params[j.src_off + (long)n * j.s_n + (long)k * j.s_k + t];
        if (j.scale_off >= 0) v *= wn_scale[j.scale_off + n];
      }
      tile[(nl * TAPS + t) * TP + kl] = v;
    }
  }
  __syncthreads();
  const int ldA = TAPS * j.A_inner_pad, ldB = TAPS * j.B_inner_pad;
  for (int e = threadIdx.x; e < total / 4; e += 256) {
    const int kl = (e % (TE / 4)) * 4, rest = e / (TE / 4);
    const int t = rest % TAPS, nl = rest / TAPS;
    const int n = n0 + nl, k = k0 + kl;
    if (n < j.A_rows_pad && k < j.A_inner_pad) {
      pack_t o;
#pragma unroll
      for (int q = 0; q < 4; ++q) o[q] = ET<T>::from_f32(tile[(nl * TAPS + t) * TP + kl + q]);
      const long off = j.frag_tiled ? tiled_offset<T>(n, t * j.A_inner_pad + k, ldA) : (long)n * ldA + t * j.A_inner_pad + k;
      *reinterpret_cast<pack_t*>(shadow + j.dstA + off) = o;
    }
  }
  for (int e = threadIdx.x; j.dstB >= 0 && e < total / 4; e += 256) {
    const int nl = (e % (TE / 4)) * 4, rest = e / (TE / 4);
    const int t = rest % TAPS, kl = rest / TAPS;
    const int n = n0 + nl, k = k0 + kl;
    if (k < j.B_rows_pad && n < j.B_inner_pad) {
      pack_t o;
      const bool live = k < j.B_rows_real;
#pragma unroll
      for (int q = 0; q < 4; ++q) o[q] = ET<T>::from_f32(live ? tile[((nl + q) * TAPS + t) * TP + kl] : 0.f);
      const long off = j.frag_tiled ? tiled_offset<T>(k, t * j.B_inner_pad + n, ldB) : (long)k * ldB + t * j.B_inner_pad + n;
      *reinterpret_cast<pack_t*>(shadow + j.dstB + off) = o;
    }
  }
}

template <typename T>
__global__ __launch_bounds__(256) void relayout_kernel(const float* __restrict__ params, T* __restrict__ shadow,
                                                       const float* __restrict__ wn_scale, const RelayoutJob* __restrict__ jobs,
                                                       int njobs, const int* __restrict__ block_job, int block_base, int nblocks) {
  __shared__ __attribute__((aligned(16))) float tile[32 * 33 * 9];
  for (int bid = (int)blockIdx.x + block_base; bid < block_base + nblocks; bid += (int)gridDim.x) {
    int lo = 0;
    if (block_job) {
      lo = block_job[bid];
    } else {
      int hi = njobs - 1;
      while (lo < hi) {
        const int mid = (lo + hi + 1) >> 1;
        if (jobs[mid].block_start <= bid) lo = mid; else hi = mid - 1;
      }
    }
    const RelayoutJob j = jobs[lo];
    const int t_id = bid - j.block_start;
    const int n0 = (t_id / j.tiles_k) * j.tile, k0 = (t_id % j.tiles_k) * j.tile;
    if (j.taps == 1) relayout_tile<T, 1, 64>(j, params, shadow, wn_scale, n0, k0, tile);
    else if (j.taps == 9) relayout_tile<T, 9, 32>(j, params, shadow, wn_scale, n0, k0, tile);
    else relayout_tile<T, 6, 32>(j, params, shadow, wn_scale, n0, k0, tile);
    __syncthreads();
  }
}

struct WnJob { long v_off, g_off, out_off; int rows, K; int row_start; };

__global__ void wn_scale_kernel(const float* __restrict__ params, float* __restrict__ scale, float* __restrict__ inv_norm,
                                const WnJob* __restrict__ jobs, int njobs, int row_base, int total_rows) {
  const int grow = row_base + blockIdx.x * (blockDim.x >> 6) + (threadIdx.x >> 6);
  if (grow >= row_base + total_rows) return;
  int lo = 0, hi = njobs - 1;
  while (lo < hi) {
    const int mid = (lo + hi + 1) >> 1;
    if (jobs[mid].row_start <= grow) lo = mid; else hi = mid - 1;
  }
  const WnJob j = jobs[lo];
  const int row = grow - j.row_start, lane = threadIdx.x & 63;
// ... 205 lines not shown
    if (t2 < end) load(t2, RA);
    process(RB);
    if (t2 >= end) break;
    t = t2;
  }
}

template <typename T>
__global__ __launch_bounds__(256) void adam_cast_kernel(float* __restrict__ p, const float* __restrict__ g, float* __restrict__ m,
                                                        float* __restrict__ v, float* __restrict__ vmax, T* __restrict__ shadow,
                                                        const AdamTileJob* __restrict__ jobs, int njobs, int chunk_begin, int nchunks, AdamHyper h) {
  typedef typename RPack4<T>::type pack_t;
  for (int c = chunk_begin + (int)blockIdx.x; c < chunk_begin + nchunks; c += (int)gridDim.x) {
    int lo = 0, hi = njobs - 1;
    while (lo < hi) {
      const int mid = (lo + hi + 1) >> 1;
      if (jobs[mid].tile_start <= c) lo = mid; else hi = mid - 1;
    }
    const AdamTileJob j = jobs[lo];
    const long rel = (long)(c - j.tile_start) * 4096 + threadIdx.x * 4;
    f32x4 pp[4], gg[4], mm[4], vv[4], vx[4];
#pragma unroll
    for (int q = 0; q < 4; ++q) {
      const long i = j.src_off + rel + q * 1024;
      pp[q] = ld_stream<kNtCast>(p + i); gg[q] = ld_stream<kNtCast>(g + i);
      mm[q] = ld_stream<kNtCast>(m + i); vv[q] = ld_stream<kNtCast>(v + i);
      vx[q] = ld_stream<kNtCast>(vmax + i);
    }
#pragma unroll
    for (int q = 0; q < 4; ++q) {
      adam_amsgrad_update4(pp[q], gg[q], mm[q], vv[q], vx[q], h);
      const long i = j.src_off + rel + q * 1024;
      st_stream<kNtCast>(p + i, pp[q]); st_stream<kNtCast>(m + i, mm[q]);
      st_stream<kNtCast>(v + i, vv[q]); st_stream<kNtCast>(vmax + i, vx[q]);
      pack_t o;
#pragma unroll
      for (int k = 0; k < 4; ++k) o[k] = ET<T>::from_f32(pp[q][k]);
      *reinterpret_cast<pack_t*>(shadow + j.dstA + rel + q * 1024) = o;
    }
  }
}

struct AdamSeg { long off, len; };
__global__ void adam_amsgrad_seg_kernel(float* __restrict__ p, const float* __restrict__ g, float* __restrict__ m, float* __restrict__ v,
                                        float* __restrict__ vmax, const AdamSeg* __restrict__ segs, int s0, long begin, long end,
                                        AdamHyper h) {
  const AdamSeg sg = segs[s0 + blockIdx.y];
  const long lo = sg.off > begin ? sg.off : begin, hi = sg.off + sg.len < end ? sg.off + sg.len : end;
  const long stride = (long)gridDim.x * blockDim.x * 4;
  for (long i0 = lo + ((long)blockIdx.x * blockDim.x + threadIdx.x) * 4; i0 < hi; i0 += 4 * stride) {
    if (i0 + 3 * stride + 3 < hi) {
      f32x4 pp[4], gg[4], mm[4], vv[4], vx[4];
#pragma unroll
      for (int q = 0; q < 4; ++q) {
        const long i = i0 + q * stride;
        pp[q] = ld_stream<kNtSeg>(p + i); gg[q] = ld_stream<kNtSeg>(g + i);
        mm[q] = ld_stream<kNtSeg>(m + i); vv[q] = ld_stream<kNtSeg>(v + i); vx[q] = ld_stream<kNtSeg>(vmax + i);
      }
#pragma unroll
      for (int q = 0; q < 4; ++q) {
        const long i = i0 + q * stride;
        adam_amsgrad_update4(pp[q], gg[q], mm[q], vv[q], vx[q], h);
        st_stream<kNtSeg>(p + i, pp[q]); st_stream<kNtSeg>(m + i, mm[q]);
        st_stream<kNtSeg>(v + i, vv[q]); st_stream<kNtSeg>(vmax + i, vx[q]);
      }
      continue;
    }
    for (int q = 0; q < 4; ++q) {
      const long i = i0 + q * stride;
      if (i + 3 < hi) {
        f32x4 pp = *reinterpret_cast<f32x4*>(p + i), gg = *reinterpret_cast<const f32x4*>(g + i);
        f32x4 mm = *reinterpret_cast<f32x4*>(m + i), vv = *reinterpret_cast<f32x4*>(v + i);
        f32x4 vx = *reinterpret_cast<f32x4*>(vmax + i);
        adam_amsgrad_update4(pp, gg, mm, vv, vx, h);
        *reinterpret_cast<f32x4*>(p + i) = pp; *reinterpret_cast<f32x4*>(m + i) = mm;
        *reinterpret_cast<f32x4*>(v + i) = vv; *reinterpret_cast<f32x4*>(vmax + i) = vx;
      } else {
        for (long k = i; k < hi; ++k) adam_amsgrad_update(p[k], g[k], m[k], v[k], vmax[k], h);
      }
    }
  }
}

}

using namespace ipoke;

extern "C" int ipoke_adam_tile_job_size(void) { return (int)sizeof(AdamTileJob); }
extern "C" int ipoke_adam_seg_size(void) { return (int)sizeof(AdamSeg); }

static AdamHyper make_hyper(float lr, float beta1, float beta2, float eps, float wd, int step, float grad_scale) {
  return adam_make_hyper(lr, beta1, beta2, eps, wd, step, grad_scale);
}

extern "C" int ipoke_adam_amsgrad_shadow_tiles(float* p, const float* g, float* m, float* v, float* vmax, void* shadow, const void* jobs_dev,
                                               int njobs, int tile_begin, int ntiles, float lr, float beta1, float beta2, float eps,
                                               float weight_decay, int step, float grad_scale, int max_blocks, int dtype, void* stream) {
  IPK_REQUIRE(p && g && m && v && vmax && shadow && jobs_dev && njobs >= 1 && ntiles >= 0 && step >= 1, "bad arguments");
  IPK_REQUIRE(dtype == IPOKE_BF16 || dtype == IPOKE_F32, "bad dtype");
  if (ntiles == 0) return IPOKE_OK;
  const AdamHyper h = make_hyper(lr, beta1, beta2, eps, weight_decay, step, grad_scale);
  const int grid = max_blocks > 0 && max_blocks < ntiles ? max_blocks : ntiles;
  hipStream_t s = reinterpret_cast<hipStream_t>(stream);
  if (dtype == IPOKE_BF16)
    hipLaunchKernelGGL(adam_shadow_tile_kernel<bf16_t>, dim3(grid), dim3(256), 0, s, p, g, m, v, vmax, (bf16_t*)shadow,
                       (const AdamTileJob*)jobs_dev, njobs, tile_begin, ntiles, h);
  else
    hipLaunchKernelGGL(adam_shadow_tile_kernel<float>, dim3(grid), dim3(256), 0, s, p, g, m, v, vmax, (float*)shadow,
                       (const AdamTileJob*)jobs_dev, njobs, tile_begin, ntiles, h);
  IPK_LAUNCH_CHECK();
  return IPOKE_OK;
}

extern "C" int ipoke_adam_amsgrad_cast_tiles(float* p, const float* g, float* m, float* v, float* vmax, void* shadow, const void* jobs_dev,
                                             int njobs, int tile_begin, int ntiles, float lr, float beta1, float beta2, float eps,
                                             float weight_decay, int step, float grad_scale, int max_blocks, int dtype, void* stream) {
  IPK_REQUIRE(p && g && m && v && vmax && shadow && jobs_dev && njobs >= 1 && ntiles >= 0 && step >= 1, "bad arguments");
  IPK_REQUIRE(dtype == IPOKE_BF16 || dtype == IPOKE_F32, "bad dtype");
  if (ntiles == 0) return IPOKE_OK;
  const AdamHyper h = make_hyper(lr, beta1, beta2, eps, weight_decay, step, grad_scale);
  const int cap = max_blocks > 0 ? max_blocks : 4096;
  const int grid = cap < ntiles ? cap : ntiles;
  hipStream_t s = reinterpret_cast<hipStream_t>(stream);
  if (dtype == IPOKE_BF16)
    hipLaunchKernelGGL(adam_cast_kernel<bf16_t>, dim3(grid), dim3(256), 0, s, p, g, m, v, vmax, (bf16_t*)shadow, (const AdamTileJob*)jobs_dev, njobs,
                       tile_begin, ntiles, h);
  else
    hipLaunchKernelGGL(adam_cast_kernel<float>, dim3(grid), dim3(256), 0, s, p, g, m, v, vmax, (float*)shadow, (const AdamTileJob*)jobs_dev, njobs,
                       tile_begin, ntiles, h);
  IPK_LAUNCH_CHECK();
  return IPOKE_OK;
}

extern "C" int ipoke_adam_amsgrad_segments(float* p, const float* g, float* m, float* v, float* vmax, const void* segs_dev, int seg_begin,
                                           int nsegs, int64_t begin, int64_t end, float lr, float beta1, float beta2, float eps,
                                           float weight_decay, int step, float grad_scale, int blocks_per_segment, void* stream) {
  IPK_REQUIRE(p && g && m && v && vmax && segs_dev && nsegs >= 0 && seg_begin >= 0 && end >= begin && step >= 1, "bad arguments");
  if (nsegs == 0) return IPOKE_OK;
  const AdamHyper h = make_hyper(lr, beta1, beta2, eps, weight_decay, step, grad_scale);
  hipLaunchKernelGGL(adam_amsgrad_seg_kernel, dim3(blocks_per_segment > 0 ? blocks_per_segment : 8, nsegs), dim3(256), 0,
                     reinterpret_cast<hipStream_t>(stream), p, g, m, v, vmax, (const AdamSeg*)segs_dev, seg_begin, (long)begin, (long)end, h);
  IPK_LAUNCH_CHECK();
  return IPOKE_OK;
}

extern "C" int ipoke_relayout_job_size(void) { return (int)sizeof(RelayoutJob); }
extern "C" int ipoke_wn_job_size(void) { return (int)sizeof(WnJob); }

extern "C" int ipoke_relayout_multi(const float* params, void* shadow, const float* wn_scale, const void* jobs_dev, int njobs,
                                    int total_blocks, const int32_t* block_job_dev, int dtype, void* stream) {
  return ipoke_relayout_multi_range(params, shadow, wn_scale, jobs_dev, njobs, 0, total_blocks, block_job_dev, dtype, stream);
}
extern "C" int ipoke_relayout_multi_range(const float* params, void* shadow, const float* wn_scale, const void* jobs_dev, int njobs,
                                          int block_begin, int nblocks, const int32_t* block_job_dev, int dtype, void* stream) {
  IPK_REQUIRE(params && shadow && jobs_dev && njobs > 0 && nblocks >= 0 && block_begin >= 0, "bad arguments");
  if (nblocks == 0) return IPOKE_OK;
  hipStream_t s = reinterpret_cast<hipStream_t>(stream);
  static const int cap_env = getenv("IPOKE_RELAYOUT_BLOCKS") ? atoi(getenv("IPOKE_RELAYOUT_BLOCKS")) : 0;
  const int cap = block_begin == 0 && nblocks > 100000 ? 65536 : (cap_env > 0 ? cap_env : nblocks);
  const int grid = nblocks < cap ? nblocks : cap;
  if (dtype == IPOKE_BF16)
    hipLaunchKernelGGL(relayout_kernel<bf16_t>, dim3(grid), dim3(256), 0, s, params, (bf16_t*)shadow, wn_scale,
                       (const RelayoutJob*)jobs_dev, njobs, block_job_dev, block_begin, nblocks);
  else
    hipLaunchKernelGGL(relayout_kernel<float>, dim3(grid), dim3(256), 0, s, params, (float*)shadow, wn_scale,
                       (const RelayoutJob*)jobs_dev, njobs, block_job_dev, block_begin, nblocks);
  IPK_LAUNCH_CHECK();
  return IPOKE_OK;
}
extern "C" int ipoke_wn_scale_multi(const float* params, float* scale, float* inv_norm, const void* jobs_dev, int njobs,
                                    int total_rows, void* stream) {
  return ipoke_wn_scale_multi_range(params, scale, inv_norm, jobs_dev, 0, njobs, 0, total_rows, stream);
}
extern "C" int ipoke_wn_scale_multi_range(const float* params, float* scale, float* inv_norm, const void* jobs_dev, int job_begin,
                                          int njobs, int row_begin, int nrows, void* stream) {
  IPK_REQUIRE(params && scale && inv_norm && jobs_dev && njobs >= 0 && nrows >= 0, "bad arguments");
  if (njobs == 0 || nrows == 0) return IPOKE_OK;
  hipLaunchKernelGGL(wn_scale_kernel, dim3(ceil_div(nrows, 4)), dim3(256), 0, reinterpret_cast<hipStream_t>(stream),
                     params, scale, inv_norm, (const WnJob*)jobs_dev + job_begin, njobs, row_begin, nrows);
  IPK_LAUNCH_CHECK();
  return IPOKE_OK;
}
extern "C" int ipoke_wn_bwd_multi(const float* params, float* grads, const float* inv_norm, const void* jobs_dev, int njobs,
                                  int total_rows, void* stream) {
  IPK_REQUIRE(params && grads && inv_norm && jobs_dev && njobs > 0, "bad arguments");
  hipLaunchKernelGGL(wn_bwd_kernel, dim3(ceil_div(total_rows, 4)), dim3(256), 0, reinterpret_cast<hipStream_t>(stream),
                     params, grads, inv_norm, (const WnJob*)jobs_dev, njobs, 0, total_rows);
  IPK_LAUNCH_CHECK();
  return IPOKE_OK;
}
extern "C" int ipoke_wn_bwd_multi_range(const float* params, float* grads, const float* inv_norm, const void* jobs_dev, int job_begin,
                                        int njobs, int row_begin, int nrows, void* stream) {
  IPK_REQUIRE(params && grads && inv_norm && jobs_dev && njobs >= 0 && nrows >= 0, "bad arguments");
  if (njobs == 0 || nrows == 0) return IPOKE_OK;
  hipLaunchKernelGGL(wn_bwd_kernel, dim3(ceil_div(nrows, 4)), dim3(256), 0, reinterpret_cast<hipStream_t>(stream),
                     params, grads, inv_norm, (const WnJob*)jobs_dev + job_begin, njobs, row_begin, nrows);
  IPK_LAUNCH_CHECK();
  return IPOKE_OK;
}
```

Baseline: 6598 video-frames/sec.

## Fuse weight-norm backward, AMSGrad update and relayout into one optimizer pass

Adds a one-pass optimizer path for the flow. One kernel folds the weight-norm gradient into the Adam/AMSGrad update, also runs Adam on the plain parameter segments, and recomputes the new norm scales. A second kernel applies Adam to tap-sized conv weights while relaying them into the bf16 shadow. This replaces separate wn_bwd, adam and relayout passes that each read params and grads again. It is on by default when the tables qualify, and it adds complex segment bookkeeping that could break if the tensor-range logic is wrong.

```diff
diff --git a/include/ipoke_hip_dev.h b/include/ipoke_hip_dev.h
--- a/include/ipoke_hip_dev.h
+++ b/include/ipoke_hip_dev.h
@@ -33,6 +33,17 @@
 
 int ipoke_gru_set_fused(int mode);
 
+int ipoke_wn_adam_seg_size(void);
+int ipoke_wn_adam_multi(float* p, float* g, float* m, float* v, float* vmax, float* scale, float* inv_norm, const void* wjobs_dev, int nwjobs,
+                        const int* row_lo3, const int* nrow3, const void* segs_dev, int nsegs, const int* chunk_lo3, const int* nchunk3,
+                        float lr, float beta1, float beta2, float eps, float weight_decay, int step, float grad_scale, void* stream);
+int ipoke_relayout_adam_multi(float* p, const float* g, float* m, float* v, float* vmax, void* shadow, const float* wn_scale,
+                              const void* jobs_dev, const int32_t* block_job_dev, const int* block_lo3, const int* nblock3, float lr,
+                              float beta1, float beta2, float eps, float weight_decay, int step, float grad_scale, int dtype, void* stream);
+int ipoke_flow_wn_adam_range(ipoke_flow* f, float* params, float* grads, float* m, float* v, float* vmax, void* shadow, int64_t begin,
+                             int64_t end, float lr, float beta1, float beta2, float eps, float weight_decay, int step, float grad_scale,
+                             int fused, void* stream);
+
 #ifdef __cplusplus
 }
 #endif
diff --git a/ipoke_amd/_lib.py b/ipoke_amd/_lib.py
--- a/ipoke_amd/_lib.py
+++ b/ipoke_amd/_lib.py
@@ -254,6 +254,13 @@
     "ipoke_adam_amsgrad_segments": (c_int, [_P, _P, _P, _P, _P, _P, c_int, c_int, c_int64, c_int64, c_float, c_float, c_float, c_float,
                                             c_float, c_int, c_float, c_int, _P]),
     "ipoke_wn_bwd_multi_range": (c_int, [_P, _P, _P, _P, c_int, c_int, c_int, c_int, _P]),
+    "ipoke_wn_adam_seg_size": (c_int, []),
+    "ipoke_wn_adam_multi": (c_int, [_P, _P, _P, _P, _P, _P, _P, _P, c_int, _P, _P, _P, c_int, _P, _P, c_float, c_float, c_float, c_float,
+                                    c_float, c_int, c_float, _P]),
+    "ipoke_relayout_adam_multi": (c_int, [_P, _P, _P, _P, _P, _P, _P, _P, _P, _P, _P, c_float, c_float, c_float, c_float, c_float, c_int,
+                                          c_float, c_int, _P]),
+    "ipoke_flow_wn_adam_range": (c_int, [_P, _P, _P, _P, _P, _P, _P, c_int64, c_int64, c_float, c_float, c_float, c_float, c_float, c_int,
+                                         c_float, c_int, _P]),
     "ipoke_flow_backward_pieces": (c_int, [_P, _P, _P, _P, _P, _P, c_int, _P, _P, _P, c_int, _P, GRAD_READY_FN, _P, _P]),
     "ipoke_video_to_cl": (c_int, [_P, c_int64, c_int64, c_int64, c_int64, c_int64, c_int, c_int, c_int, c_int, c_int, _P, c_int, c_int, c_int,
                                   c_int, _P, _P]),
diff --git a/ipoke_amd/csrc/flow_engine.hip b/ipoke_amd/csrc/flow_engine.hip
--- a/ipoke_amd/csrc/flow_engine.hip
+++ b/ipoke_amd/csrc/flow_engine.hip
@@ -1,3 +1,5 @@
+#include <algorithm>
+#include <atomic>
 #include <functional>
 #include <memory>
 #include <vector>
@@ -50,11 +52,12 @@
 
 struct RelayoutJobH {
   long src_off, s_n, s_k, dstA, dstB, scale_off;
-  int taps, n_real, k_real, A_rows_pad, A_inner_pad, B_rows_pad, B_inner_pad, B_rows_real, tile, tiles_k, block_start, frag_tiled;
+  int taps, n_real, k_real, A_rows_pad, A_inner_pad, B_rows_pad, B_inner_pad, B_rows_real, tile, tiles_k, block_start, frag_tiled, adam;
 };
 struct WnJobH { long v_off, g_off, out_off; int rows, K, row_start; };
 struct AdamTileJobH { long src_off, dstA, dstB; int N, K, tile_start, pad; };
 struct AdamSegH { long off, len; };
+struct WnAdamSegH { long off, len; int chunk_start, pad; };
 struct LsRefH { long off; int C; };
 struct LuJobH { long p_l, p_u, p_logs, b_perm, b_sign, b_lmask, b_umask, b_eye, w_off; int C, pad; };
 
@@ -82,6 +85,7 @@
   std::vector<AdamSegH> asegs;
   void* d_ajobs = nullptr; void* d_rjobs2 = nullptr; void* d_rblockjob2 = nullptr; void* d_asegs = nullptr;
   std::vector<WnJobH> wjobs;
+  std::vector<WnAdamSegH> fsegs; int fchunks = 0; void* d_fsegs = nullptr; bool wn_fused = false;
   std::vector<LsRefH> lsrefs;
   void* d_rjobs = nullptr; void* d_wjobs = nullptr; void* d_lsrefs = nullptr; void* d_rblockjob = nullptr;
   hipStream_t side = nullptr;
@@ -158,7 +162,7 @@
     const int n_ext = std::max(A_rows_pad, B_inner_pad), k_ext = std::max(A_inner_pad, B_rows_pad);
     const int tiles_n = (n_ext + tile - 1) / tile, tiles_k = (k_ext + tile - 1) / tile;
     RelayoutJobH j{src, s_n, s_k, dstA, dstB, scale, taps, n_real, k_real, A_rows_pad, A_inner_pad, B_rows_pad, B_inner_pad,
-                   B_rows_real, tile, tiles_k, f.rblocks, frag_tiled};
+                   B_rows_real, tile, tiles_k, f.rblocks, frag_tiled, 0};
     f.rjobs.push_back(j);
     f.rblocks += tiles_n * tiles_k;
     const bool fusable = taps == 1 && scale < 0 && !frag_tiled && s_k == 1 && s_n == k_real && n_real % 64 == 0 && k_real % 64 == 0 &&
@@ -169,6 +173,7 @@
       f.atiles += (n_real / 64) * (k_real / 64);
     } else {
       j.block_start = f.rblocks2;
+      j.adam = scale < 0 && taps > 1;
       f.rjobs2.push_back(j);
       f.rblocks2 += tiles_n * tiles_k;
     }
@@ -666,6 +671,47 @@
 
 }
 
+static void build_fused_segments(ipoke_flow& f) {
+  std::vector<std::pair<int64_t, int64_t>> out;
+  bool ok = !f.wjobs.empty();
+  for (const auto& a : f.ajobs) out.push_back({a.src_off, a.src_off + (int64_t)a.N * a.K});
+  for (const auto& w : f.wjobs) {
+    ok = ok && w.K % 4 == 0 && w.v_off % 4 == 0 && (w.K / 4 + 127) / 128 <= 96;
+    out.push_back({w.v_off, w.v_off + (int64_t)w.rows * w.K});
+    out.push_back({w.g_off, w.g_off + w.rows});
+  }
+  for (const auto& j : f.rjobs2) {
+    if (j.adam) out.push_back({j.src_off, j.src_off + (int64_t)j.n_real * j.s_n});
+    else ok = ok && j.scale_off >= 0;
+  }
+  for (auto& o : out) o.second = align_up(o.second, 4);
+  std::sort(out.begin(), out.end());
+  for (size_t k = 1; k < out.size(); ++k) ok = ok && out[k].first >= out[k - 1].second;
+  std::vector<std::pair<int64_t, int64_t>> regions;
+  for (const auto& u : f.units) {
+    regions.push_back({u.p_lo, u.p_hi});
+    if (u.p2_lo >= 0) regions.push_back({u.p2_lo, u.p2_hi});
+  }
+  std::sort(regions.begin(), regions.end());
+  f.fsegs.clear(); f.fchunks = 0;
+  size_t x = 0;
+  for (const auto& r : regions) {
+    int64_t pos = r.first;
+    while (x < out.size() && out[x].second <= r.first) ++x;
+    for (size_t y = x; pos < r.second; ++y) {
+      const int64_t stop = y < out.size() && out[y].first < r.second ? out[y].first : r.second;
+      if (stop > pos) {
+        ok = ok && pos % 4 == 0 && stop % 4 == 0;
+        f.fsegs.push_back({(long)pos, (long)(stop - pos), f.fchunks, 0});
+        f.fchunks += (int)((stop - pos + 4095) / 4096);
+      }
+      if (y >= out.size() || out[y].first >= r.second) break;
+      pos = out[y].second;
+    }
+  }
+  f.wn_fused = ok;
+}
+
 extern "C" int ipoke_flow_create(const ipoke_flow_config* cfg, ipoke_flow** out) {
   IPK_REQUIRE(cfg && out, "null argument");
   IPK_REQUIRE(cfg->dtype == IPOKE_F32 || cfg->dtype == IPOKE_BF16, "bad dtype");
@@ -692,6 +738,7 @@
     if (pos < f->n_params) f->asegs.push_back({(long)pos, (long)(f->n_params - pos)});
     for (size_t k = 1; k < f->rjobs.size(); ++k) IPK_REQUIRE(f->rjobs[k].src_off > f->rjobs[k - 1].src_off, "relayout jobs must be in parameter order");
   }
+  build_fused_segments(*f);
   const char* env = getenv("IPOKE_NO_SIDE_STREAM");
   f->use_side = !(env && env[0] == '1');
   const char* gr = getenv("IPOKE_GRAPH");
@@ -782,6 +829,11 @@
     IPK_HIP(hipMalloc(&f->d_rblockjob2, bj.size() * sizeof(int32_t)));
     IPK_HIP(hipMemcpy(f->d_rblockjob2, bj.data(), bj.size() * sizeof(int32_t), hipMemcpyHostToDevice));
   }
+  IPK_REQUIRE((int)sizeof(WnAdamSegH) == ipoke_wn_adam_seg_size(), "segment table layout mismatch");
+  if (!f->fsegs.empty()) {
+    IPK_HIP(hipMalloc(&f->d_fsegs, f->fsegs.size() * sizeof(WnAdamSegH)));
+    IPK_HIP(hipMemcpy(f->d_fsegs, f->fsegs.data(), f->fsegs.size() * sizeof(WnAdamSegH), hipMemcpyHostToDevice));
+  }
   IPK_HIP(hipMalloc(&f->d_wjobs, f->wjobs.size() * sizeof(WnJobH)));
   IPK_HIP(hipMemcpy(f->d_wjobs, f->wjobs.data(), f->wjobs.size() * sizeof(WnJobH), hipMemcpyHostToDevice));
   if (!f->lujobs.empty()) {
@@ -814,6 +866,7 @@
   if (f->d_rblockjob) (void)hipFree(f->d_rblockjob);
   if (f->d_ajobs) (void)hipFree(f->d_ajobs);
   if (f->d_asegs) (void)hipFree(f->d_asegs);
+  if (f->d_fsegs) (void)hipFree(f->d_fsegs);
   if (f->d_rjobs2) (void)hipFree(f->d_rjobs2);
   if (f->d_rblockjob2) (void)hipFree(f->d_rblockjob2);
   if (f->d_w1tab) (void)hipFree(f->d_w1tab);
@@ -1001,6 +1054,87 @@
     if (rc) return rc;
   }
   return prepare_range(f, params, shadow, begin, end, true, stream);
+}
+
+namespace ipoke { std::atomic<int> g_wn_adam_mode{1}; }
+
+static int wn_adam_ranges(ipoke_flow* f, float* params, float* grads, float* m, float* v, float* vmax, void* shadow, const int64_t* b,
+                          const int64_t* e, float lr, float beta1, float beta2, float eps, float weight_decay, int step, float grad_scale,
+                          int max_blocks, void* stream, bool skip_tiles) {
+  IPK_REQUIRE(f->wn_fused, "this flow's tables do not qualify for the one-pass optimizer");
+  float* wn_scale = reinterpret_cast<float*>(shadow);
+  float* wn_inv = wn_scale + align_up(f->wn_rows, 64);
+  void* sh = reinterpret_cast<unsigned char*>(shadow) + 2 * align_up(f->wn_rows, 64) * 4;
+  int row_lo[3] = {0, 0, 0}, nrow[3] = {0, 0, 0}, ch_lo[3] = {0, 0, 0}, nch[3] = {0, 0, 0}, bl_lo[3] = {0, 0, 0}, nbl[3] = {0, 0, 0};
+  for (int q = 0; q < 3; ++q) {
+    if (b[q] < 0 || e[q] <= b[q]) continue;
+    int a0 = 0;
+    while (a0 < (int)f->ajobs.size() && f->ajobs[a0].src_off < b[q]) ++a0;
+    int a1 = a0;
+    while (a1 < (int)f->ajobs.size() && f->ajobs[a1].src_off < e[q]) ++a1;
+    if (a1 > a0 && !skip_tiles) {
+      IPK_REQUIRE(f->ajobs[a1 - 1].src_off + (int64_t)f->ajobs[a1 - 1].N * f->ajobs[a1 - 1].K <= e[q], "range must cover whole tensors");
+      const int t0 = f->ajobs[a0].tile_start, t1 = a1 < (int)f->ajobs.size() ? f->ajobs[a1].tile_start : f->atiles;
+      int rc = f->c2_straight
+          ? ipoke_adam_amsgrad_cast_tiles(params, grads, m, v, vmax, sh, f->d_ajobs, (int)f->ajobs.size(), t0, t1 - t0, lr, beta1, beta2,
+                                          eps, weight_decay, step, grad_scale, max_blocks, f->cfg.dtype, stream)
+          : ipoke_adam_amsgrad_shadow_tiles(params, grads, m, v, vmax, sh, f->d_ajobs, (int)f->ajobs.size(), t0, t1 - t0, lr, beta1, beta2,
+                                            eps, weight_decay, step, grad_scale, max_blocks, f->cfg.dtype, stream);
+      if (rc) return rc;
+    }
+    int w0 = 0;
+    while (w0 < (int)f->wjobs.size() && f->wjobs[w0].v_off < b[q]) ++w0;
+    int w1 = w0;
+    while (w1 < (int)f->wjobs.size() && f->wjobs[w1].v_off < e[q]) ++w1;
+    if (w1 > w0) {
+      row_lo[q] = f->wjobs[w0].row_start;
+      nrow[q] = (w1 < (int)f->wjobs.size() ? f->wjobs[w1].row_start : (int)f->wn_rows) - row_lo[q];
+    }
+    int s0 = 0;
+    while (s0 < (int)f->fsegs.size() && f->fsegs[s0].off < b[q]) ++s0;
+    int s1 = s0;
+    while (s1 < (int)f->fsegs.size() && f->fsegs[s1].off < e[q]) ++s1;
+    if (s1 > s0) {
+      IPK_REQUIRE(f->fsegs[s1 - 1].off + f->fsegs[s1 - 1].len <= e[q], "range must cover whole tensors");
+      ch_lo[q] = f->fsegs[s0].chunk_start;
+      nch[q] = (s1 < (int)f->fsegs.size() ? f->fsegs[s1].chunk_start : f->fchunks) - ch_lo[q];
+    }
+    int j0 = 0;
+    while (j0 < (int)f->rjobs2.size() && f->rjobs2[j0].src_off < b[q]) ++j0;
+    int j1 = j0;
+    while (j1 < (int)f->rjobs2.size() && f->rjobs2[j1].src_off < e[q]) ++j1;
+    if (j1 > j0) {
+      bl_lo[q] = f->rjobs2[j0].block_start;
+      nbl[q] = (j1 < (int)f->rjobs2.size() ? f->rjobs2[j1].block_start : f->rblocks2) - bl_lo[q];
+    }
+  }
+  int rc = ipoke_wn_adam_multi(params, grads, m, v, vmax, wn_scale, wn_inv, f->d_wjobs, (int)f->wjobs.size(), row_lo, nrow, f->d_fsegs,
+                               (int)f->fsegs.size(), ch_lo, nch, lr, beta1, beta2, eps, weight_decay, step, grad_scale, stream);
+  if (rc) return rc;
+  return ipoke_relayout_adam_multi(params, grads, m, v, vmax, sh, wn_scale, f->d_rjobs2, reinterpret_cast<const int32_t*>(f->d_rblockjob2),
+                                   bl_lo, nbl, lr, beta1, beta2, eps, weight_decay, step, grad_scale, f->cfg.dtype, stream);
+}
+
+extern "C" int ipoke_flow_wn_adam_range(ipoke_flow* f, float* params, float* grads, float* m, float* v, float* vmax, void* shadow,
+                                        int64_t begin, int64_t end, float lr, float beta1, float beta2, float eps, float weight_decay,
+                                        int step, float grad_scale, int fused, void* stream) {
+  IPK_REQUIRE(f && params && grads && m && v && vmax && shadow && begin >= 0 && end >= begin && end <= f->n_params, "bad arguments");
+  { int rc0 = ensure_device(f); if (rc0) return rc0; }
+  if (fused) {
+    const int64_t b[3] = {begin, -1, -1}, e[3] = {end, -1, -1};
+    return wn_adam_ranges(f, params, grads, m, v, vmax, shadow, b, e, lr, beta1, beta2, eps, weight_decay, step, grad_scale, 0, stream, false);
+  }
+  int w0 = 0;
+  while (w0 < (int)f->wjobs.size() && f->wjobs[w0].v_off < begin) ++w0;
+  int w1 = w0;
+  while (w1 < (int)f->wjobs.size() && f->wjobs[w1].v_off < end) ++w1;
+  if (w1 > w0) {
+    const int row0 = f->wjobs[w0].row_start, row1 = w1 < (int)f->wjobs.size() ? f->wjobs[w1].row_start : (int)f->wn_rows;
+    const float* wn_inv = reinterpret_cast<const float*>(shadow) + align_up(f->wn_rows, 64);
+    int rc = ipoke_wn_bwd_multi_range(params, grads, wn_inv, f->d_wjobs, w0, w1 - w0, row0, row1 - row0, stream);
+    if (rc) return rc;
+  }
+  return adam_range(f, params, grads, m, v, vmax, shadow, begin, end, lr, beta1, beta2, eps, weight_decay, step, grad_scale, 0, stream);
 }
 
 static int make_lanes(const Ctx& full, int want, std::vector<Ctx>& lanes) {
@@ -1516,13 +1650,15 @@
       p1[k] = un.p_hi; wj1[k] = un.wj_hi; rw1[k] = un.row_hi;
       if (un.p2_lo >= 0) { if (p0[2] < 0) p0[2] = un.p2_lo; p1[2] = un.p2_hi; }
     }
-    for (int kind = 0; kind < 2; ++kind) {
+    static const bool probe_skip_adam = getenv("IPOKE_PROBE_SKIP_ADAM") != nullptr;
+    const bool one_pass = f->nadam.on && !probe_skip_adam && !ready && f->c2_straight && f->wn_fused &&
+                          g_wn_adam_mode.load(std::memory_order_relaxed) != 0;
+    for (int kind = 0; kind < 2 && !one_pass; ++kind) {
       if (p0[kind] < 0) continue;
       r = ipoke_wn_bwd_multi_range(params, grads, c.wn_inv(), f->d_wjobs, wj0[kind], wj1[kind] - wj0[kind], rw0[kind],
                                    rw1[kind] - rw0[kind], rstream);
       if (r) return r;
     }
-    static const bool probe_skip_adam = getenv("IPOKE_PROBE_SKIP_ADAM") != nullptr;
     if (f->nadam.on && !probe_skip_adam) {
       ipoke_flow::NativeAdam A = f->nadam;
       {
@@ -1530,9 +1666,15 @@
         static const int late = getenv("IPOKE_ADAM_LATE_PIECES") ? atoi(getenv("IPOKE_ADAM_LATE_PIECES")) : 3;
         if (early > 0 && piece < (int)pieces.size() - late) A.max_blocks = early;
       }
-      for (int kind = 0; kind < 3; ++kind) {
-        if (p0[kind] < 0 || p1[kind] <= p0[kind]) continue;
-        r = native_adam_range(p0[kind], p1[kind], A.max_blocks); if (r) return r;
+      if (one_pass) {
+        r = wn_adam_ranges(f, const_cast<float*>(params), grads, A.m, A.v, A.vmax, const_cast<void*>(shadow), p0, p1, A.lr, A.beta1, A.beta2,
+                           A.eps, A.wd, A.step, A.grad_scale, A.max_blocks, rstream, wgrad_adam);
+        if (r) return r;
+      } else {
+        for (int kind = 0; kind < 3; ++kind) {
+          if (p0[kind] < 0 || p1[kind] <= p0[kind]) continue;
+          r = native_adam_range(p0[kind], p1[kind], A.max_blocks); if (r) return r;
+        }
       }
     }
     if (ready)
diff --git a/ipoke_amd/csrc/gemm.hip b/ipoke_amd/csrc/gemm.hip
--- a/ipoke_amd/csrc/gemm.hip
+++ b/ipoke_amd/csrc/gemm.hip
@@ -2320,6 +2320,7 @@
 }
 
 static std::atomic<int> g_c64_mode{-1}, g_halo16_mode{-1};
+extern std::atomic<int> g_wn_adam_mode;
 static int dispatch_mode(std::atomic<int>& slot, const char* env_name) {
   int m = slot.load(std::memory_order_relaxed);
   if (m < 0) {
@@ -3828,8 +3829,12 @@
 
 extern "C" int ipoke_set_dispatch_override(const char* name, int value) {
   IPK_REQUIRE(name != nullptr && value <= 2, "bad arguments");
+  if (!strcmp(name, "wn_adam")) {
+    g_wn_adam_mode.store(value == 0 ? 0 : 1, std::memory_order_relaxed);
+    return IPOKE_OK;
+  }
   std::atomic<int>* slot = !strcmp(name, "c64") ? &g_c64_mode : (!strcmp(name, "halo16") ? &g_halo16_mode : nullptr);
-  IPK_REQUIRE(slot != nullptr, "unknown dispatch switch (c64 | halo16)");
+  IPK_REQUIRE(slot != nullptr, "unknown dispatch switch (c64 | halo16 | wn_adam)");
   slot->store(value < 0 ? -1 : value, std::memory_order_relaxed);
   return IPOKE_OK;
 }
diff --git a/ipoke_amd/csrc/prep.hip b/ipoke_amd/csrc/prep.hip
--- a/ipoke_amd/csrc/prep.hip
+++ b/ipoke_amd/csrc/prep.hip
@@ -12,7 +12,10 @@
   int tile, tiles_k;
   int block_start;
   int frag_tiled;
+  int adam;
 };
+
+struct AdamPtrs { float* p; const float* g; float* m; float* v; float* vmax; AdamHyper h; };
 
 template <typename T>
 __device__ __forceinline__ long tiled_offset(int row, int col, int ld) {
@@ -25,9 +28,10 @@
 template <> struct RPack4<bf16_t> { typedef __attribute__((ext_vector_type(4))) __bf16 type; };
 template <> struct RPack4<float> { typedef f32x4 type; };
 
-template <typename T, int TAPS, int TE>
+template <typename T, int TAPS, int TE, bool ADAM = false>
 __device__ __forceinline__ void relayout_tile(const RelayoutJob& j, const float* __restrict__ params, T* __restrict__ shadow,
-                                              const float* __restrict__ wn_scale, int n0, int k0, float* tile) {
+                                              const float* __restrict__ wn_scale, int n0, int k0, float* tile,
+                                              const AdamPtrs* A = nullptr) {
   constexpr int TP = TE + 1;
   constexpr int total = TE * TE * TAPS;
   typedef typename RPack4<T>::type pack_t;
@@ -47,6 +51,39 @@
       }
 #pragma unroll
       for (int q = 0; q < 4; ++q) tile[nl * TP + kl + q] = v[q];
+    }
+  } else if (ADAM && j.adam) {
+    static_assert(total % 1024 == 0, "whole rounds");
+    for (int e0 = threadIdx.x; e0 < total; e0 += 1024) {
+      float pp[4], gg[4], mm[4], vv[4], vx[4];
+      long idx[4]; int tl[4];
+      bool live[4];
+#pragma unroll
+      for (int q = 0; q < 4; ++q) {
+        const int e = e0 + 256 * q;
+        const int t = e % TAPS, rest = e / TAPS;
+        const int m = rest % TE, sl = rest / TE;
+        const int nl = k_mid ? sl : m, kl = k_mid ? m : sl;
+        const int n = n0 + nl, k = k0 + kl;
+        tl[q] = (nl * TAPS + t) * TP + kl;
+        live[q] = n < j.n_real && k < j.k_real;
+        idx[q] = j.src_off + (long)n * j.s_n + (long)k * j.s_k + t;
+        pp[q] = gg[q] = mm[q] = vv[q] = vx[q] = 0.f;
+        if (live[q]) {
+          pp[q] = __builtin_nontemporal_load(A->p + idx[q]); gg[q] = __builtin_nontemporal_load(A->g + idx[q]);
+          mm[q] = __builtin_nontemporal_load(A->m + idx[q]); vv[q] = __builtin_nontemporal_load(A->v + idx[q]);
+          vx[q] = __builtin_nontemporal_load(A->vmax + idx[q]);
+        }
+      }
+#pragma unroll
+      for (int q = 0; q < 4; ++q) {
+        if (live[q]) {
+          adam_amsgrad_update(pp[q], gg[q], mm[q], vv[q], vx[q], A->h);
+          __builtin_nontemporal_store(pp[q], A->p + idx[q]); __builtin_nontemporal_store(mm[q], A->m + idx[q]);
+          __builtin_nontemporal_store(vv[q], A->v + idx[q]); __builtin_nontemporal_store(vx[q], A->vmax + idx[q]);
+        }
+        tile[tl[q]] = pp[q];
+      }
     }
   } else {
     for (int e = threadIdx.x; e < total; e += 256) {
@@ -418,6 +455,170 @@
   }
 }
 
+struct WnAdamSeg { long off, len; int chunk_start, pad; };
+struct Span3 { int lo[3], n[3]; };
+static constexpr int kWnAdamMaxIt = 96;
+
+__device__ __forceinline__ int span3_at(const Span3& s, int r) {
+  if (r < s.n[0]) return s.lo[0] + r;
+  r -= s.n[0];
+  if (r < s.n[1]) return s.lo[1] + r;
+  return s.lo[2] + r - s.n[1];
+}
+
+__device__ __forceinline__ float wn_term(bool short_row, bool h0, bool h1, const f32x4& a0, const f32x4& b0, const f32x4& a1, const f32x4& b1) {
+#pragma clang fp contract(off)
+  if (!h0) return 0.f;
+  float e = short_row ? fmaf(a0[3], b0[3], fmaf(a0[2], b0[2], fmaf(a0[0], b0[0], a0[1] * b0[1])))
+                      : ((a0[0] * b0[0] + a0[1] * b0[1]) + a0[2] * b0[2]) + a0[3] * b0[3];
+  if (h1) {
+    e = e + a1[0] * b1[0];
+    e = e + a1[1] * b1[1];
+    e = e + a1[2] * b1[2];
+    e = e + a1[3] * b1[3];
+  }
+  return e;
+}
+__device__ __forceinline__ float wn_sq_term(bool h0, bool h1, const f32x4& a, const f32x4& b) {
+  return wn_term(false, h0, h1, a, a, b, b);
+}
+__device__ __forceinline__ float wn_dv(float a, float d, float bcoef, float v) {
+#pragma clang fp contract(off)
+  return fmaf(a, d, -(bcoef * v));
+}
+
+__global__ __launch_bounds__(256) void wn_adam_kernel(float* __restrict__ params, float* __restrict__ grads, float* __restrict__ m,
+                                                      float* __restrict__ v, float* __restrict__ vmax, float* __restrict__ scale,
+                                                      float* __restrict__ inv_norm, const WnJob* __restrict__ jobs, int njobs, Span3 rows,
+                                                      int nrows, const WnAdamSeg* __restrict__ segs, int nsegs, Span3 chunks, AdamHyper h) {
+  __shared__ float part[kWnAdamMaxIt * 64];
+  const int tid = threadIdx.x, lane = tid & 63, w = tid >> 6;
+  if ((int)blockIdx.x >= nrows) {
+    const int c = span3_at(chunks, (int)blockIdx.x - nrows);
+    int lo = 0, hi = nsegs - 1;
+    while (lo < hi) {
+      const int mid = (lo + hi + 1) >> 1;
+      if (segs[mid].chunk_start <= c) lo = mid; else hi = mid - 1;
+    }
+    const WnAdamSeg sg = segs[lo];
+    const long rel = (long)(c - sg.chunk_start) * 4096 + tid * 4;
+    f32x4 pp[4], gg[4], mm[4], vv[4], vx[4];
+#pragma unroll
+    for (int q = 0; q < 4; ++q) {
+      if (rel + q * 1024 < sg.len) {
+        const long i = sg.off + rel + q * 1024;
+        pp[q] = ld_stream<kNtSeg>(params + i); gg[q] = ld_stream<kNtSeg>(grads + i);
+        mm[q] = ld_stream<kNtSeg>(m + i); vv[q] = ld_stream<kNtSeg>(v + i); vx[q] = ld_stream<kNtSeg>(vmax + i);
+      }
+    }
+#pragma unroll
+    for (int q = 0; q < 4; ++q) {
+      if (rel + q * 1024 < sg.len) {
+        const long i = sg.off + rel + q * 1024;
+        adam_amsgrad_update4(pp[q], gg[q], mm[q], vv[q], vx[q], h);
+        st_stream<kNtSeg>(params + i, pp[q]); st_stream<kNtSeg>(m + i, mm[q]);
+        st_stream<kNtSeg>(v + i, vv[q]); st_stream<kNtSeg>(vmax + i, vx[q]);
+      }
+    }
+    return;
+  }
+  const int grow = span3_at(rows, (int)blockIdx.x);
+  int lo = 0, hi = njobs - 1;
+  while (lo < hi) {
+    const int mid = (lo + hi + 1) >> 1;
+    if (jobs[mid].row_start <= grow) lo = mid; else hi = mid - 1;
+  }
+  const WnJob j = jobs[lo];
+  const int row = grow - j.row_start;
+  const long base = j.v_off + (long)row * j.K;
+  const int n4 = j.K >> 2, nit = (n4 + 127) >> 7;
+  const bool short_row = n4 <= 192;
+  const f32x4 z4 = {0.f, 0.f, 0.f, 0.f};
+  for (int it = w; it < nit; it += 8) {
+    f32x4 a[2][2], b[2][2];
+    bool h0[2], h1[2];
+#pragma unroll
+    for (int u = 0; u < 2; ++u) {
+      const int k = lane + 128 * (it + 4 * u);
+      h0[u] = it + 4 * u < nit && k < n4; h1[u] = it + 4 * u < nit && k + 64 < n4;
+      a[u][0] = h0[u] ? *reinterpret_cast<const f32x4*>(params + base + 4L * k) : z4;
+      b[u][0] = h0[u] ? *reinterpret_cast<const f32x4*>(grads + base + 4L * k) : z4;
+      a[u][1] = h1[u] ? *reinterpret_cast<const f32x4*>(params + base + 4L * (k + 64)) : z4;
+      b[u][1] = h1[u] ? *reinterpret_cast<const f32x4*>(grads + base + 4L * (k + 64)) : z4;
+    }
+#pragma unroll
+    for (int u = 0; u < 2; ++u)
+      if (it + 4 * u < nit) part[(it + 4 * u) * 64 + lane] = wn_term(short_row, h0[u], h1[u], a[u][0], b[u][0], a[u][1], b[u][1]);
+  }
+  __syncthreads();
+  float dot = 0.f;
+  for (int it = 0; it < nit; ++it) dot += part[it * 64 + lane];
+  dot = wave_sum(dot);
+  const float inv = inv_norm[j.out_off + row], g = params[j.g_off + row];
+  const float a = g * inv, bcoef = g * dot * inv * inv * inv;
+  __syncthreads();
+  for (int it = w; it < nit; it += 4) {
+    const int k = lane + 128 * it;
+    const bool h0 = k < n4, h1 = k + 64 < n4;
+    f32x4 pp[2], dd[2], mm[2], vv[2], vx[2];
+#pragma unroll
+    for (int q = 0; q < 2; ++q) {
+      pp[q] = dd[q] = mm[q] = vv[q] = vx[q] = z4;
+      if (q ? h1 : h0) {
+        const long i = base + 4L * (k + 64 * q);
+        pp[q] = *reinterpret_cast<const f32x4*>(params + i); dd[q] = *reinterpret_cast<const f32x4*>(grads + i);
+        mm[q] = ld_stream<kNtSeg>(m + i); vv[q] = ld_stream<kNtSeg>(v + i); vx[q] = ld_stream<kNtSeg>(vmax + i);
+      }
+    }
+#pragma unroll
+    for (int q = 0; q < 2; ++q) {
+      f32x4 o;
+#pragma unroll
+      for (int r = 0; r < 4; ++r) o[r] = wn_dv(a, dd[q][r], bcoef, pp[q][r]);
+      if (q ? h1 : h0) {
+        const long i = base + 4L * (k + 64 * q);
+        adam_amsgrad_update4(pp[q], o, mm[q], vv[q], vx[q], h);
+        st_stream<kNtSeg>(grads + i, o);
+        st_stream<kNtSeg>(params + i, pp[q]); st_stream<kNtSeg>(m + i, mm[q]);
+        st_stream<kNtSeg>(v + i, vv[q]); st_stream<kNtSeg>(vmax + i, vx[q]);
+      }
+    }
+    part[it * 64 + lane] = wn_sq_term(h0, h1, pp[0], pp[1]);
+  }
+  __syncthreads();
+  if (w == 0) {
+    float s = 0.f;
+    for (int it = 0; it < nit; ++it) s += part[it * 64 + lane];
+    s = wave_sum(s);
+    if (lane == 0) {
+      const float dg = dot * inv;
+      const long gi = j.g_off + row;
+      float gp = g, gm = m[gi], gv = v[gi], gx = vmax[gi];
+      grads[gi] = dg;
+      adam_amsgrad_update(gp, dg, gm, gv, gx, h);
+      params[gi] = gp; m[gi] = gm; v[gi] = gv; vmax[gi] = gx;
+      const float nrm = sqrtf(s);
+      scale[j.out_off + row] = gp / nrm;
+      inv_norm[j.out_off + row] = 1.f / nrm;
+    }
+  }
+}
+
+template <typename T>
+__global__ __launch_bounds__(256) void relayout_adam_kernel(float* __restrict__ params, T* __restrict__ shadow, const float* __restrict__ wn_scale,
+                                                            const RelayoutJob* __restrict__ jobs, const int* __restrict__ block_job, Span3 blocks,
+                                                            AdamPtrs A) {
+  __shared__ __attribute__((aligned(16))) float tile[32 * 33 * 9];
+  const int bid = span3_at(blocks, (int)blockIdx.x);
+  const RelayoutJob j = jobs[block_job[bid]];
+  const int t_id = bid - j.block_start;
+  const int n0 = (t_id / j.tiles_k) * j.tile, k0 = (t_id % j.tiles_k) * j.tile;
+  A.p = params;
+  if (j.taps == 1) relayout_tile<T, 1, 64, true>(j, params, shadow, wn_scale, n0, k0, tile, &A);
+  else if (j.taps == 9) relayout_tile<T, 9, 32, true>(j, params, shadow, wn_scale, n0, k0, tile, &A);
+  else relayout_tile<T, 6, 32, true>(j, params, shadow, wn_scale, n0, k0, tile, &A);
+}
+
 }
 
 using namespace ipoke;
@@ -480,6 +681,54 @@
   return IPOKE_OK;
 }
 
+extern "C" int ipoke_wn_adam_seg_size(void) { return (int)sizeof(WnAdamSeg); }
+
+static Span3 make_span3(const int* lo3, const int* n3, int& total) {
+  Span3 s;
+  total = 0;
+  for (int q = 0; q < 3; ++q) { s.lo[q] = lo3 ? lo3[q] : 0; s.n[q] = n3 ? n3[q] : 0; total += s.n[q]; }
+  return s;
+}
+
+extern "C" int ipoke_wn_adam_multi(float* p, float* g, float* m, float* v, float* vmax, float* scale, float* inv_norm, const void* wjobs_dev,
+                                   int nwjobs, const int* row_lo3, const int* nrow3, const void* segs_dev, int nsegs, const int* chunk_lo3,
+                                   const int* nchunk3, float lr, float beta1, float beta2, float eps, float weight_decay, int step,
+                                   float grad_scale, void* stream) {
+  IPK_REQUIRE(p && g && m && v && vmax && scale && inv_norm && step >= 1, "bad arguments");
+  int nrows = 0, nchunks = 0;
+  const Span3 rows = make_span3(row_lo3, nrow3, nrows), chunks = make_span3(chunk_lo3, nchunk3, nchunks);
+  IPK_REQUIRE(nrows >= 0 && nchunks >= 0 && (nrows == 0 || (wjobs_dev && nwjobs > 0)) && (nchunks == 0 || (segs_dev && nsegs > 0)),
+              "bad ranges");
+  if (nrows + nchunks == 0) return IPOKE_OK;
+  const AdamHyper h = make_hyper(lr, beta1, beta2, eps, weight_decay, step, grad_scale);
+  hipLaunchKernelGGL(wn_adam_kernel, dim3(nrows + nchunks), dim3(256), 0, reinterpret_cast<hipStream_t>(stream), p, g, m, v, vmax, scale,
+                     inv_norm, (const WnJob*)wjobs_dev, nwjobs, rows, nrows, (const WnAdamSeg*)segs_dev, nsegs, chunks, h);
+  IPK_LAUNCH_CHECK();
+  return IPOKE_OK;
+}
+
+extern "C" int ipoke_relayout_adam_multi(float* p, const float* g, float* m, float* v, float* vmax, void* shadow, const float* wn_scale,
+                                         const void* jobs_dev, const int32_t* block_job_dev, const int* block_lo3, const int* nblock3,
+                                         float lr, float beta1, float beta2, float eps, float weight_decay, int step, float grad_scale,
+                                         int dtype, void* stream) {
+  IPK_REQUIRE(p && g && m && v && vmax && shadow && step >= 1, "bad arguments");
+  IPK_REQUIRE(dtype == IPOKE_BF16 || dtype == IPOKE_F32, "bad dtype");
+  int nblocks = 0;
+  const Span3 blocks = make_span3(block_lo3, nblock3, nblocks);
+  IPK_REQUIRE(nblocks >= 0 && (nblocks == 0 || (jobs_dev && block_job_dev)), "bad ranges");
+  if (nblocks == 0) return IPOKE_OK;
+  const AdamPtrs A{p, g, m, v, vmax, make_hyper(lr, beta1, beta2, eps, weight_decay, step, grad_scale)};
+  hipStream_t s = reinterpret_cast<hipStream_t>(stream);
+  if (dtype == IPOKE_BF16)
+    hipLaunchKernelGGL(relayout_adam_kernel<bf16_t>, dim3(nblocks), dim3(256), 0, s, p, (bf16_t*)shadow, wn_scale,
+                       (const RelayoutJob*)jobs_dev, (const int*)block_job_dev, blocks, A);
+  else
+    hipLaunchKernelGGL(relayout_adam_kernel<float>, dim3(nblocks), dim3(256), 0, s, p, (float*)shadow, wn_scale,
+                       (const RelayoutJob*)jobs_dev, (const int*)block_job_dev, blocks, A);
+  IPK_LAUNCH_CHECK();
+  return IPOKE_OK;
+}
+
 extern "C" int ipoke_relayout_job_size(void) { return (int)sizeof(RelayoutJob); }
 extern "C" int ipoke_wn_job_size(void) { return (int)sizeof(WnJob); }
 
```

Result: no change. 6603 video-frames/sec (median of 6 runs) (+0.1%).
